# nyu-systems/CLM-GS

Measured on AMD Instinct MI355X. Metric: training images/s (Rubble-4K 28M Gaussians clm_offload), higher is better.
Workload: dtype f32

## Files before the change

### clm_gs_amd/_lib.py

```python
import ctypes
import os
import time

import torch

_HERE = os.path.dirname(os.path.abspath(__file__))
LIB_PATH = os.environ.get("CLMGS_LIB_PATH") or os.path.join(_HERE, "libclmgs_hip.so")

_vp, _i, _i64, _f, _sz = ctypes.c_void_p, ctypes.c_int, ctypes.c_int64, ctypes.c_float, ctypes.c_size_t
_d = ctypes.c_double

SIGNATURES = {
    "clmgs_version": (_i, []),
    "clmgs_last_error": (ctypes.c_char_p, []),
    "clmgs_projection_fwd": (_i, [_vp, _i, _i, _vp, _vp, _vp, _vp, _vp, _i, _i, _f, _f, _f, _f, _vp, _vp, _vp, _vp]),
    "clmgs_visibility_select_temp_bytes": (_sz, [_i, _i]),
    "clmgs_visibility_select_count": (_i, [_vp, _i, _i, _vp, _vp, _vp, _vp, _vp, _i, _i, _f, _f, _f, _f, _vp, _sz, _vp]),
    "clmgs_visibility_select_count_blocks": (_i, [_vp, _i, _i, _vp, _vp, _vp, _vp, _vp, _i, _i, _f, _f, _f, _f, _vp, _sz, _vp, _vp]),
    "clmgs_visibility_select_emit": (_i, [_vp, _i, _i, _vp, _vp]),
    "clmgs_visibility_raw": (_i, [_vp, _i, _i, _vp, _vp, _vp, _vp, _vp, _i, _i, _f, _f, _f, _f, _vp]),
    "clmgs_projection_bwd": (_i, [_vp, _i, _i, _vp, _vp, _vp, _vp, _vp, _i, _i, _f, _vp, _vp, _vp, _vp, _vp, _vp, _vp]),
    "clmgs_sh_fwd": (_i, [_vp, _i, _i, _vp, _vp, _vp, _vp]),
    "clmgs_sh_bwd": (_i, [_vp, _i, _i, _vp, _vp, _vp, _vp, _vp, _i, _vp]),
    "clmgs_isect_count_temp_bytes": (_sz, [_i]),
    "clmgs_isect_count": (_i, [_vp, _i, _i, _vp, _vp, _i, _i, _i, _vp, _vp, _vp, _sz]),
    "clmgs_isect_sort_temp_bytes": (_sz, [_i64]),
    "clmgs_isect_emit_sort": (_i, [_vp, _i, _i, _i64, _vp, _vp, _vp, _vp, _i, _i, _i, _vp, _vp, _vp, _sz]),
    "clmgs_isect_offsets": (_i, [_vp, _i64, _vp, _i, _i, _i, _vp]),
    "clmgs_isect2_order_temp_bytes": (_sz, [_i]),
    "clmgs_isect2_order_count": (_i, [_vp, _i, _vp, _vp, _vp, _i, _i, _i, _vp, _vp, _vp, _vp, _vp, _vp, _sz, _vp]),
    "clmgs_isect2_sort_temp_bytes": (_sz, [_i64]),
    "clmgs_isect2_emit_sort": (_i, [_vp, _i, _i64, _vp, _vp, _vp, _vp, _i, _i, _vp, _vp, _vp, _vp, _vp, _sz, _vp]),
    "clmgs_isect2_emit_sort_dev": (_i, [_vp, _i, _i64, _vp, _vp, _vp, _vp, _vp, _i, _i, _vp, _vp, _vp, _vp, _vp, _sz, _vp]),
    "clmgs_isect3_front_temp_bytes": (_sz, [_i, _i]),
    "clmgs_isect3_front": (_i, [_vp, _i, _vp, _vp, _i, _i, _i, _vp, _vp, _vp, _vp, _sz]),
    "clmgs_isect3_bin_temp_bytes": (_sz, [_i64, _i]),
    "clmgs_isect3_bin": (_i, [_vp, _i, _i64, _vp, _i, _i, _vp, _vp, _vp, _vp, _vp, _vp, _vp, _sz]),
    "clmgs_isect3_bin_dev": (_i, [_vp, _i, _i64, _vp, _vp, _i, _i, _vp, _vp, _vp, _vp, _vp, _vp, _vp, _sz]),
    "clmgs_rasterize_fwd_dev": (_i, [_vp, _i, _i, _i64, _vp, _vp, _i, _i, _i, _i, _i, _vp, _vp, _vp, _vp, _vp, _vp]),
    "clmgs_rasterize_bwd_dev": (_i, [_vp, _i, _i, _i64, _vp, _vp, _vp, _i, _i, _i, _i, _i, _vp, _vp, _vp, _vp, _vp, _vp, _vp, _vp, _vp]),
    "clmgs_rasterize_pack_bytes": (_sz, [_i, _i]),
    "clmgs_rasterize_fwd": (_i, [_vp, _i, _i, _i64, _vp, _vp, _vp, _vp, _vp, _i, _i, _i, _i, _i, _vp, _vp, _vp, _vp, _vp, _vp]),
    "clmgs_rasterize_partials_bytes": (_sz, [_i64]),
    "clmgs_rasterize_bwd": (_i, [_vp, _i, _i, _i64, _vp, _vp, _i, _i, _i, _i, _i, _vp, _vp, _vp, _vp, _vp, _vp, _vp, _vp, _vp, _vp, _vp, _vp, _vp, _vp]),
    "clmgs_rasterize4_fwd": (_i, [_vp, _i, _i, _i64, _vp, _vp, _vp, _vp, _vp, _i, _i, _i, _i, _i, _vp, _vp, _vp, _vp, _vp, _vp]),
    "clmgs_rasterize4_bwd": (_i, [_vp, _i, _i, _i64, _vp, _vp, _i, _i, _i, _i, _i, _vp, _vp, _vp, _vp, _vp, _vp, _vp, _vp, _vp, _vp, _vp, _vp, _vp, _vp]),
    "clmgs_preprocess_fwd": (_i, [_vp, _i, _vp, _vp, _vp, _vp, _vp, _vp, _i, _vp, _vp, _vp, _i, _i, _i, _f, _f, _f, _f, _vp, _vp, _vp, _vp, _vp, _vp, _vp, _vp]),
    "clmgs_preprocess_bwd": (_i, [_vp, _i, _vp, _vp, _vp, _vp, _vp, _vp, _i, _vp, _vp, _vp, _i, _i, _i, _f, _vp, _vp, _vp, _vp, _vp, _vp, _vp, _vp, _vp, _vp, _vp, _i, _vp, _vp, _vp, _vp, _i]),
    "clmgs_ssim_fwd": (_i, [_vp, _i, _i, _i, _i, _vp, _vp, _vp, _vp, _vp, _vp]),
    "clmgs_ssim_bwd": (_i, [_vp, _i, _i, _i, _i, _vp, _vp, _vp, _f, _vp, _vp, _vp, _vp]),
    "clmgs_loss_slots": (_i, []),
    "clmgs_l1_ssim_loss_fwd": (_i, [_vp, _i, _i, _vp, _i64, _i64, _i64, _vp, _vp, _vp, _vp, _vp]),
    "clmgs_l1_ssim_loss_bwd": (_i, [_vp, _i, _i, _vp, _i64, _i64, _i64, _vp, _vp, _f, _vp, _vp, _vp, _vp]),
    "clmgs_rows_gather": (_i, [_vp, _vp, _vp, _vp, _vp, _i, _i64, _i, _i]),
    "clmgs_rows_scatter_add": (_i, [_vp, _vp, _vp, _vp, _vp, _i, _i64, _i, _i]),
    "clmgs_scatter_to_bit": (_i, [_vp, _vp, _i, _vp, _i64, _i]),
    "clmgs_extract_ffs": (_i, [_vp, _vp, _i, _i64, _vp]),
    "clmgs_pair_overlap_count": (_i, [_vp, _vp, _i, _i64, _i, _vp]),
    "clmgs_set_signal": (_i, [_vp, _vp, _i, ctypes.c_int32]),
    "clmgs_adam_rows": (_i, [_vp, _vp, _vp, _vp, _vp, _vp, _i, _vp, _i64, _i, _vp, _d, _d, _d, _i, _i, _f, _i]),
    "clmgs_pack_small": (_i, [_vp, _i64, _vp, _vp, _vp, _vp, _vp]),
    "clmgs_adam_small_packed": (_i, [_vp, _i64, _vp, _vp, _vp, _vp, _vp, _vp, _d, _d, _d, _i, _i, _f, _vp, _i]),
    "clmgs_adam_catch_up": (_i, [_vp, _vp, _vp, _vp, _vp, _vp, _i, _i64, _i, _vp, _d, _d, _d, _i, _i, _i, _vp, _vp, _f, _i]),
    "clmgs_host_adam_rows": (_i, [_vp, _vp, _vp, _vp, _vp, _i64, _i, _vp, _d, _d, _d, _i, _i, _f, _i, _vp, _i]),
    "clmgs_host_pool_start": (_i, [_i]),
    "clmgs_host_usable_cpus": (_i, []),
    "clmgs_memcpy_async": (_i, [_vp, _vp, _vp, _sz, _i]),
    "clmgs_host_rows_prepare": (_i, [_vp, _vp, _vp, _vp, _vp, _vp, _vp, _i64, _i, _vp, _d, _d, _d, _i, _i, _i, _f, _i, _vp, _i]),
    "clmgs_densify_stats": (_i, [_vp, _i64, _vp, _vp, _vp, _i, _f, _f, _vp, _vp, _vp]),
    "clmgs_morton_order_temp_bytes": (_sz, [_i64]),
    "clmgs_morton_order": (_i, [_vp, _i64, _vp, _vp, _vp, _vp, _sz]),
    "clmgs_tsp_tour": (_i, [_i, _vp, _vp]),
    "clmgs_knn3_mean_dist2": (_i, [_vp, _i, _vp, _vp, _f, _f, _f, _f, _i, _i, _i, _i, _vp]),
    "clmgs_host_groups_temp_bytes": (_sz, [_i64]),
    "clmgs_host_groups": (_i, [_vp, _i64, _vp, _vp, _i, _i, _vp, _i, _vp, _vp, _vp, _vp, _vp, _sz]),
    "clmgs_publish_pack": (_i, [_vp, _vp, _vp, _vp, _vp, _i, _i64, _i64, _i64, _i]),
    "clmgs_visibility_candidates": (_i, [_vp, _i, _i, _i, _i, _vp, _vp, _vp, _vp, _i, _i, _f, _f, _f, _f, _f, _vp]),
    "clmgs_small_rows_scatter": (_i, [_vp, _i64, _vp, _vp, _vp, _vp, _vp, _vp, _vp]),
    "clmgs_adam_small_packed_range": (_i, [_vp, _i64, _i64, _i64, _vp, _vp, _vp, _vp, _vp, _vp, _d, _d, _d, _i, _i, _f, _vp, _i]),
    "clmgs_small_deferred_kmax": (_i, []),
    "clmgs_adam_small_deferred": (_i, [_vp, _i64, _vp, _vp, _vp, _vp, _vp, _vp, _vp, _i, _i, _vp, _vp, _vp, _vp, _d, _d, _d,
                                       _f, _i, _vp, _vp, _i, _i, _f, _f, _f, _i, _vp]),
    "clmgs_device_errors": (_i, [_vp, _i]),
    "clmgs_pinned_alloc": (_vp, [_sz]),
    "clmgs_pinned_free": (_i, [_vp]),
}

_lib = None

TIMING = None
STATS = {"n_isects": [], "n_emitted": [], "host_wait_s": 0.0}


class ClmgsError(RuntimeError):
    pass


class _Entry:

    def __init__(self, name, fn, takes_stream):
        self.name, self.fn, self.takes_stream = name, fn, takes_stream

    def __call__(self, *args):
        if TIMING is None or not self.takes_stream:
            return self.fn(*args)
        s, e = torch.cuda.Event(enable_timing=True), torch.cuda.Event(enable_timing=True)
        h = getattr(args[0], "value", args[0])
        st = torch.cuda.ExternalStream(h) if h else torch.cuda.current_stream()
        s.record(st)
        rc = self.fn(*args)
        e.record(st)
        TIMING.setdefault(self.name, []).append((s, e))
        return rc


class _Namespace:
    pass


_NO_STREAM = {"clmgs_version", "clmgs_loss_slots", "clmgs_small_deferred_kmax", "clmgs_isect3_front_temp_bytes",
              "clmgs_isect3_bin_temp_bytes", "clmgs_last_error", "clmgs_isect_count_temp_bytes",
              "clmgs_isect_sort_temp_bytes", "clmgs_host_groups_temp_bytes", "clmgs_isect2_order_temp_bytes", "clmgs_isect2_sort_temp_bytes", "clmgs_visibility_select_temp_bytes", "clmgs_rasterize_pack_bytes", "clmgs_rasterize_partials_bytes", "clmgs_host_adam_rows", "clmgs_host_pool_start", "clmgs_host_usable_cpus", "clmgs_host_rows_prepare", "clmgs_tsp_tour",
              "clmgs_pinned_alloc", "clmgs_pinned_free", "clmgs_device_errors"}


def timing_summary():
    out = {}
    for name, evs in (TIMING or {}).items():
        out[name] = (len(evs), sum(s.elapsed_time(e) for s, e in evs))
    return out


def lib():
    global _lib
    if _lib is None:
        if not os.path.exists(LIB_PATH):
            raise ClmgsError(
                f"{LIB_PATH} not found: build it with `python -c 'import __graft_entry__ as g; g.build()'` "
                "(make -C clm_gs_amd/csrc).  clm_gs_amd has no CPU/eager fallback."
            )
        l = ctypes.CDLL(LIB_PATH)
        ns = _Namespace()
        for name, (res, args) in SIGNATURES.items():
            fn = getattr(l, name)
            fn.restype = res
            fn.argtypes = args
            setattr(ns, name, _Entry(name, fn, name not in _NO_STREAM))
        _lib = ns
    return _lib


def check(rc):
    if rc != 0:
        msg = lib().clmgs_last_error()
        raise ClmgsError(f"libclmgs_hip error {rc}: {msg.decode() if msg else ''}")


def check_device_errors():
    bits = ctypes.c_uint32(0)
    check(lib().clmgs_device_errors(ctypes.byref(bits), 1))
    if bits.value & 4:
        raise ClmgsError("deferred small-attribute Adam: a block of rows was further behind than the recorded step history "
                         "(clmgs_adam_small_deferred, device error bit 4): its parameters are wrong")
    if bits.value:
        raise ClmgsError(f"device error word {bits.value}: no kernel of this library raises that value (4 is the only one "
                         "in use); the results since the last check cannot be trusted")


HOST_REGIONS = None
REGION_TRACE = None
_ROCTX = None


def roctx():
    global _ROCTX
    if _ROCTX is None:
        _ROCTX = False
        if os.environ.get("CLMGS_ROCTX") == "1":
            for name in ("librocprofiler-sdk-roctx.so", "libroctx64.so"):
                try:
                    l = ctypes.CDLL(name)
                    l.roctxRangePushA.argtypes = [ctypes.c_char_p]
                    l.roctxRangePushA.restype = ctypes.c_int
                    l.roctxRangePop.restype = ctypes.c_int
                    _ROCTX = l
                    break
                except (OSError, AttributeError):
                    continue
    return _ROCTX


class host_region:
    __slots__ = ("name", "t0", "rx")

    def __init__(self, name):
        self.name = name

    def __enter__(self):
        self.rx = roctx()
        if self.rx:
            self.rx.roctxRangePushA(self.name.encode())
        if HOST_REGIONS is not None:
            self.t0 = time.perf_counter()

    def __exit__(self, *exc):
        if HOST_REGIONS is not None:
            dt = time.perf_counter() - self.t0
            HOST_REGIONS[self.name] = HOST_REGIONS.get(self.name, 0.0) + dt
            if REGION_TRACE is not None:
                REGION_TRACE.setdefault(self.name, []).append(round(dt * 1e3, 2))
        if self.rx:
            self.rx.roctxRangePop()
        return False


def stream():
    return ctypes.c_void_p(torch.cuda.current_stream().cuda_stream)


def dptr(t, dtype=None, allow_none=False, allow_host=False):
    if t is None:
        if allow_none:
            return None
        raise ClmgsError("required tensor is None")
    if dtype is not None and t.dtype != dtype:
        raise ClmgsError(f"expected dtype {dtype}, got {t.dtype}")
    if not t.is_contiguous():
        raise ClmgsError("tensor must be contiguous")
    if not t.is_cuda:
        if not (allow_host and (t.is_pinned() or getattr(t, "_clmgs_pinned", False))):
            raise ClmgsError("tensor must live on the GPU (no CPU fallback in clm_gs_amd)")
    return ctypes.c_void_p(t.data_ptr())
```

### clm_gs_amd/clm_kernels.py

```python
import ctypes

import torch

from . import _lib, utils
from ._lib import check, dptr, stream

F32, I32, I64, U8 = torch.float32, torch.int32, torch.int64, torch.uint8


class _FusedSSIM(torch.autograd.Function):
    @staticmethod
    def forward(ctx, img1, img2):
        L = _lib.lib()
        img1, img2 = img1.contiguous(), img2.contiguous()
        B, CH, H, W = img1.shape
        need = img1.requires_grad
        ssim_sum = torch.zeros((1024,), dtype=F32, device=img1.device)
        maps = [torch.empty_like(img1) for _ in range(3)] if need else [None, None, None]
        check(L.clmgs_ssim_fwd(stream(), B, CH, H, W, dptr(img1, F32), dptr(img2, F32),
                               dptr(ssim_sum), dptr(maps[0], F32, True), dptr(maps[1], F32, True),
                               dptr(maps[2], F32, True)))
        ctx.shape = (B, CH, H, W)
        if need:
            ctx.save_for_backward(img1, img2, *maps)
        return ssim_sum.sum() / float(img1.numel())

    @staticmethod
    def backward(ctx, v):
        L = _lib.lib()
        img1, img2, m0, m1, m2 = ctx.saved_tensors
        B, CH, H, W = ctx.shape
        v_img1 = torch.empty_like(img1)
        v = v.reshape(1).to(F32).contiguous()
        check(L.clmgs_ssim_bwd(stream(), B, CH, H, W, dptr(img1), dptr(img2), dptr(v, F32),
                               1.0 / float(img1.numel()), dptr(m0), dptr(m1), dptr(m2),
                               dptr(v_img1)))
        return v_img1, None


def fused_ssim(img1, img2):
    return _FusedSSIM.apply(img1, img2)


class _FusedL1SSIMLoss(torch.autograd.Function):
    @staticmethod
    def forward(ctx, image, gt_u8, lambda_dssim):
        L = _lib.lib()
        assert image.dim() == 3 and image.shape[0] == 3 and image.dtype == F32 and image.is_cuda
        _, H, W = image.shape
        gt_u8 = gt_u8.contiguous()
        assert gt_u8.dtype == U8 and gt_u8.shape == image.shape
        need = image.requires_grad
        slots = L.clmgs_loss_slots()
        partials = torch.zeros((slots, 2), dtype=F32, device=image.device)
        maps = torch.empty((3, 3, H, W), dtype=F32, device=image.device) if need else None
        sc, sy, sx = image.stride()
        check(L.clmgs_l1_ssim_loss_fwd(stream(), H, W, ctypes.c_void_p(image.data_ptr()), sc, sy, sx,
                                       dptr(gt_u8, U8), dptr(partials),
                                       dptr(maps[0] if need else None, F32, True),
                                       dptr(maps[1] if need else None, F32, True),
                                       dptr(maps[2] if need else None, F32, True)))
        tot = partials.sum(dim=0) / float(image.numel())
        ctx.lam = float(lambda_dssim)
        if need:
            ctx.save_for_backward(image, gt_u8, maps)
        return (1.0 - ctx.lam) * tot[0] + ctx.lam * (1.0 - tot[1])

    @staticmethod
    def backward(ctx, v):
        L = _lib.lib()
        image, gt_u8, maps = ctx.saved_tensors
        _, H, W = image.shape
        v = v.reshape(1).to(F32).contiguous()
        v_img = torch.empty_strided(image.shape, image.stride(), dtype=F32, device=image.device)
        sc, sy, sx = image.stride()
        check(L.clmgs_l1_ssim_loss_bwd(stream(), H, W, ctypes.c_void_p(image.data_ptr()), sc, sy, sx,
                                       dptr(gt_u8, U8), dptr(v, F32), ctx.lam, dptr(maps[0]),
                                       dptr(maps[1]), dptr(maps[2]),
                                       ctypes.c_void_p(v_img.data_ptr())))
        return v_img, None, None


def fused_l1_ssim_loss(image, gt_u8, lambda_dssim=0.2):
    return _FusedL1SSIMLoss.apply(image, gt_u8, lambda_dssim)


def _idx64(t):
    return 1 if t is not None and t.dtype == I64 else 0


def _rows(fn, dst, src, dst_idx, src_idx, grid):
    L = _lib.lib()
    n = (dst_idx if dst_idx is not None else src_idx).numel() if (dst_idx is not None or src_idx is not None) else dst.shape[0]
    if dst_idx is not None and src_idx is not None and dst_idx.dtype != src_idx.dtype:
        src_idx = src_idx.to(dst_idx.dtype)
    is64 = _idx64(dst_idx if dst_idx is not None else src_idx)
    cols = src.shape[-1]
    check(getattr(L, fn)(stream(), dptr(dst, F32, allow_host=True), dptr(src, F32, allow_host=True),
                         dptr(dst_idx, None, True), dptr(src_idx, None, True), is64, int(n),
                         int(cols), int(grid)))


def send_shs2gpu_stream(shs, parameters, filter_idx, grid_size=0, block_size=256):
    _rows("clmgs_rows_gather", shs, parameters, None, filter_idx, grid_size)


def send_shs2gpu_stream_retention(shs_next, parameters, shs_retent, host_indices_to_param,
                                  rtnt_indices_to_param, param_indices_from_host,
                                  param_indices_from_rtnt, grid_size=0, block_size=256,
                                  grid_size_D=0, block_size_D=256):
    if host_indices_to_param.numel():
        _rows("clmgs_rows_gather", shs_next, parameters, param_indices_from_host,
              host_indices_to_param, grid_size)
    if rtnt_indices_to_param.numel():
        _rows("clmgs_rows_gather", shs_next, shs_retent, param_indices_from_rtnt,
              rtnt_indices_to_param, grid_size_D)


def send_shs2cpu_grad_buffer_stream(shs_grad, grad_buffer, filter_idx, accum=True, grid_size=0,
                                    block_size=256):
    _rows("clmgs_rows_scatter_add" if accum else "clmgs_rows_gather", grad_buffer, shs_grad,
          filter_idx, None, grid_size)


def send_shs2cpu_grad_buffer_stream_retention(shs_grad, grad_buffer, shs_grad_next,
                                              host_indices_from_grad, rtnt_indices_from_grad,
                                              grad_indices_to_host, grad_indices_to_rtnt,
                                              accum=True, grid_size=0, block_size=256,
                                              grid_size_D=0, block_size_D=256):
    if host_indices_from_grad.numel():
        _rows("clmgs_rows_scatter_add" if accum else "clmgs_rows_gather", grad_buffer, shs_grad,
              host_indices_from_grad, grad_indices_to_host, grid_size)
    if rtnt_indices_from_grad.numel():
        _rows("clmgs_rows_gather", shs_grad_next, shs_grad, rtnt_indices_from_grad,
              grad_indices_to_rtnt, grid_size_D)


@torch.no_grad()
def spherical_harmonics_bwd_inplace(degrees_to_use, dirs, coeffs, v_coeffs, v_colors):
    L = _lib.lib()
    n = dirs.numel() // 3
    d2, c2, vc = dirs.contiguous(), coeffs.contiguous(), v_colors.contiguous()
    v_dirs = torch.empty_like(d2)
    check(L.clmgs_sh_bwd(stream(), n, int(degrees_to_use), dptr(d2, F32), dptr(c2, F32), None,
                         dptr(vc, F32), dptr(v_coeffs, F32), 1, dptr(v_dirs)))
    return v_dirs


def scatter_to_bit(bitmap, filter_idx, bit):
    L = _lib.lib()
    check(L.clmgs_scatter_to_bit(stream(), dptr(bitmap), bitmap.element_size(),
                                 dptr(filter_idx.contiguous(), I64), filter_idx.numel(), int(bit)))


def extract_ffs(bitmap, ffs):
    L = _lib.lib()
    check(L.clmgs_extract_ffs(stream(), dptr(bitmap), bitmap.element_size(), bitmap.numel(),
                              dptr(ffs, U8)))


def compute_cnt_h(bitmap, tmp_buffer, grid_size=64, block_size=256):
    L = _lib.lib()
    bsz = tmp_buffer.shape[0] + 1
    cnt = torch.zeros((bsz - 1,), dtype=I32, device=bitmap.device)
    check(L.clmgs_pair_overlap_count(stream(), dptr(bitmap), bitmap.element_size(), bitmap.numel(),
                                     bsz, dptr(cnt)))
    tmp_buffer.zero_()
    tmp_buffer[:, 0] = cnt
    return cnt


def pair_overlap_count(bitmap, bsz):
    L = _lib.lib()
    cnt = torch.zeros((bsz - 1,), dtype=I32, device=bitmap.device)
    check(L.clmgs_pair_overlap_count(stream(), dptr(bitmap), bitmap.element_size(), bitmap.numel(),
                                     int(bsz), dptr(cnt)))
    return cnt


def set_signal(signal_tensor_pinned, idx, value):
    L = _lib.lib()
    check(L.clmgs_set_signal(stream(), ctypes.c_void_p(signal_tensor_pinned.data_ptr()), int(idx),
                             int(value)))


def selective_adam_update(param, grad, exp_avg, exp_avg_sq, visibility, lr, beta1, beta2, eps, N, M):
    L = _lib.lib()
    col_lr = torch.full((M,), float(lr), dtype=F32, device=param.device)
    vis = visibility.contiguous().view(U8)
    check(L.clmgs_adam_rows(stream(), dptr(param, F32), dptr(grad, F32), dptr(exp_avg, F32),
                            dptr(exp_avg_sq, F32), None, 0, dptr(vis, U8), int(N), int(M),
                            dptr(col_lr), float(beta1), float(beta2), float(eps), 1, 0, 1.0, 0))


def adam_rows(p, g, m, v, rows, col_lr, beta1, beta2, eps, step, bias_correction=True,
              grad_scale=1.0, zero_grad=False, mask=None):
    L = _lib.lib()
    n_rows = rows.numel() if rows is not None else p.shape[0]
    cols = p.shape[-1] if p.dim() > 1 else 1
    check(L.clmgs_adam_rows(stream(), dptr(p, F32), dptr(g, F32, True), dptr(m, F32), dptr(v, F32),
                            dptr(rows, None, True), _idx64(rows),
                            dptr(mask.view(U8) if mask is not None else None, U8, True),
                            int(n_rows), int(cols), dptr(col_lr, F32), float(beta1), float(beta2),
                            float(eps), int(step), int(bool(bias_correction)), float(grad_scale),
                            int(bool(zero_grad))))


def adam_catch_up(p, m, v, last_step, rows, col_lr, beta1, beta2, eps, to_step, bias_correction=True,
                  max_replay=256, g=None, g_step=None, grad_scale=1.0, keep_grad=False, moment_row0=0):
    L = _lib.lib()
    n_rows = rows.numel() if rows is not None else p.shape[0]
    m_ptr, v_ptr = dptr(m, F32), dptr(v, F32)
    if moment_row0:
        assert rows is not None, "a moment shard needs an explicit row list"
        back = int(moment_row0) * int(p.shape[-1]) * 4
        m_ptr, v_ptr = ctypes.c_void_p(m_ptr.value - back), ctypes.c_void_p(v_ptr.value - back)
    check(L.clmgs_adam_catch_up(stream(), dptr(p, F32), m_ptr, v_ptr, dptr(last_step, I32),
                                dptr(rows, None, True), _idx64(rows), int(n_rows), int(p.shape[-1]),
                                dptr(col_lr, F32), float(beta1), float(beta2), float(eps), int(to_step),
                                int(bool(bias_correction)), int(max_replay), dptr(g, F32, True),
                                dptr(g_step, I32, True), float(grad_scale), int(bool(keep_grad))))
    if rows is None:
        last_step[: p.shape[0]].fill_(int(to_step))
    else:
        utils.fill_rows(last_step, rows.long(), int(to_step))


def densify_stats(filter_idx, v_means2d, radii, width, height, max_radii2D, xyz_gradient_accum,
                  denom, only_visible=True):
    L = _lib.lib()
    n = radii.numel()
    check(L.clmgs_densify_stats(stream(), n, dptr(filter_idx, I64, True),
                                dptr(v_means2d.contiguous(), F32), dptr(radii.contiguous(), I32),
                                int(bool(only_visible)), float(width) * 0.5, float(height) * 0.5, dptr(max_radii2D, F32),
                                dptr(xyz_gradient_accum, F32), dptr(denom, F32)))
```

### clm_gs_amd/csrc/loss.hip

```cpp
#include "common.h"

namespace clmgs {

constexpr int LR = 5;
constexpr int LM = 2 * LR + 1;
constexpr int LS_W = 64, LS_ROWS = 62;
constexpr int LS_IN = LS_W + 2 * LR;
constexpr int LS_PITCH = LS_IN + 2;
constexpr int LS_RING = 8;
constexpr int LU = 12;
#ifndef CLMGS_LOSS_LP
#define CLMGS_LOSS_LP 4
#endif
constexpr int LP = CLMGS_LOSS_LP;
constexpr int LOSS_SLOTS = 1024;
constexpr float L_C1 = 0.01f * 0.01f, L_C2 = 0.03f * 0.03f;

constexpr float l_win[11] = {
    0.0010283801f, 0.0075987582f, 0.0360007721f, 0.1093606895f, 0.2130055377f, 0.2660117249f,
    0.2130055377f, 0.1093606895f, 0.0360007721f, 0.0075987582f, 0.0010283801f};

struct ImgView { const float* p; int64_t sc, sy, sx; };

__device__ __forceinline__ void wave_sync() {
  __builtin_amdgcn_fence(__ATOMIC_RELEASE, "wavefront");
  __builtin_amdgcn_wave_barrier();
  __builtin_amdgcn_fence(__ATOMIC_ACQUIRE, "wavefront");
}

__device__ __forceinline__ float gt_from_byte(unsigned byte) {
  const float v = (float)byte;
  const float r = 1.0f / 255.0f;
  const float q = v * r;
  return fmaf(fmaf(-q, 255.0f, v), r, q);
}

__device__ __forceinline__ bool strip_of_block(int H, int W, int& c, int& x0, int& y0, int& slot) {
  const int n_sx = (W + LS_W - 1) / LS_W, n_sy = (H + LS_ROWS - 1) / LS_ROWS;
  const int grp = blockIdx.x / 24, rem = blockIdx.x - grp * 24;
  c = rem >> 3;
  const int strip = grp * 8 + (rem & 7);
  if (strip >= n_sx * n_sy) return false;
  const int by = strip / n_sx, bx = strip - by * n_sx;
  x0 = bx * LS_W; y0 = by * LS_ROWS;
  slot = ((c * n_sy + by) * n_sx + bx) & (LOSS_SLOTS - 1);
  return true;
}

#ifndef CLMGS_LOSS_FWD_WAVES
#define CLMGS_LOSS_FWD_WAVES 3
#endif
__global__ void __launch_bounds__(64, CLMGS_LOSS_FWD_WAVES)
loss_fwd_kernel(int H, int W, ImgView img, const uint8_t* __restrict__ gt, float* __restrict__ partials,
                float* __restrict__ m1, float* __restrict__ m2, float* __restrict__ m3) {
  __shared__ float la[LS_RING][LS_PITCH], lb[LS_RING][LS_PITCH];
  const int lane = threadIdx.x;
  int c, x0, y0, slot;
  if (!strip_of_block(H, W, c, x0, y0, slot)) return;
  const size_t plane = (size_t)H * W;
  const int xo = x0 + lane;
  const int n_rows = min(LS_ROWS, H - y0) + 2 * LR;
  const int xs = x0 - LR + lane;
  const bool xs_ok = xs >= 0 && xs < W;
  const int xh = x0 - LR + LS_W + lane;
  const bool h_ok = lane < 2 * LR && xh < W;
  const float* img_c = img.p + c * img.sc;
  const uint8_t* gt_c = gt + c * plane;
  const unsigned xs_c = (unsigned)min(max(xs, 0), W - 1);
  const unsigned xh_c = (unsigned)min(x0 - LR + LS_W + min(lane, 2 * LR - 1), W - 1);
  const unsigned xs_off = xs_c * (unsigned)img.sx, xh_off = xh_c * (unsigned)img.sx;
  float pa[LP], ha[LP];
  unsigned pb[LP], hb[LP];
  auto fetch = [&](int r, int s) {
    const int y = min(max(y0 - LR + min(r, n_rows - 1), 0), H - 1);
    const float* ir = img_c + y * img.sy;
    const uint8_t* gr = gt_c + (size_t)y * W;
    pa[s] = ir[xs_off]; pb[s] = gr[xs_c];
    ha[s] = ir[xh_off]; hb[s] = gr[xh_c];
  };
#pragma unroll
  for (int s = 0; s < LP; ++s) fetch(s, s);
  float win[LU][4];
  float l1 = 0.f, ss = 0.f;
  for (int r0 = 0; r0 < n_rows; r0 += LU) {
#pragma unroll
    for (int k = 0; k < LU; ++k) {
      const int r = r0 + k;
      {
        __builtin_amdgcn_sched_barrier(0);
        const int s = k % LP, buf = r & (LS_RING - 1);
        {
          const int yin = y0 - LR + r;
          const bool row_ok = yin >= 0 && yin < H;
          const bool okm = row_ok && xs_ok, okh = row_ok && h_ok;
          la[buf][lane] = okm ? pa[s] : 0.f; lb[buf][lane] = okm ? gt_from_byte(pb[s]) : 0.f;
          if (lane < 2 * LR) {
            la[buf][LS_W + lane] = okh ? ha[s] : 0.f; lb[buf][LS_W + lane] = okh ? gt_from_byte(hb[s]) : 0.f;
          }
        }
        fetch(r + LP, s);
        wave_sync();
        float s0 = 0.f, s1 = 0.f, s2 = 0.f, s3 = 0.f;
#pragma unroll
        for (int j = 0; j < LM; ++j) {
          const float av = la[buf][lane + j], bv = lb[buf][lane + j];
          const float wa_ = l_win[j] * av, wb_ = l_win[j] * bv;
          s0 += wa_; s1 += wb_; s2 = fmaf(wa_, av, s2); s2 = fmaf(wb_, bv, s2); s3 = fmaf(wa_, bv, s3);
        }
        win[k][0] = s0; win[k][1] = s1; win[k][2] = s2; win[k][3] = s3;
        {
          float acc[4];
#pragma unroll
          for (int q = 0; q < 4; ++q) {
            float sacc = 0.f;
#pragma unroll
            for (int j = 0; j < LM; ++j) sacc += l_win[j] * win[(k + 2 + j) % LU][q];
            acc[q] = sacc;
          }
          const int y = y0 + r - 2 * LR;
          const bool out_ok = (r >= 2 * LR) && (r < n_rows) && (xo < W) && (y < H);
          {
            const float mu1 = acc[0], mu2 = acc[1];
            const float mu1sq = mu1 * mu1, mu2sq = mu2 * mu2, mu12 = mu1 * mu2;
            const float sgs = (acc[2] - mu1sq) - mu2sq, sg12 = acc[3] - mu12;
            const float A = 2.f * mu12 + L_C1, B = 2.f * sg12 + L_C2;
            const float D = mu1sq + mu2sq + L_C1, E = sgs + L_C2;
            const float iDE = __builtin_amdgcn_rcpf(D * E);
            const float val = A * B * iDE;
            ss += out_ok ? val : 0.f;
            const int cbuf = (r - LR) & (LS_RING - 1);
            l1 += out_ok ? fabsf(la[cbuf][lane + LR] - lb[cbuf][lane + LR]) : 0.f;
            if (m1 && out_ok) {
              const float d_mu1 = 2.f * mu2 * B * iDE - val * 2.f * mu1 * __builtin_amdgcn_rcpf(D);
              const float d_s1 = -val * __builtin_amdgcn_rcpf(E), d_s12 = 2.f * A * iDE;
              const size_t orow = c * plane + (size_t)y * W;
              (m1 + orow)[(unsigned)xo] = d_mu1 - 2.f * mu1 * d_s1 - mu2 * d_s12;
              (m2 + orow)[(unsigned)xo] = d_s1; (m3 + orow)[(unsigned)xo] = d_s12;
            }
          }
        }
      }
    }
  }
  const float tl1 = wave_sum(l1), tss = wave_sum(ss);
  if (lane == 0) {
    atomicAdd(partials + 2 * slot, tl1);
    atomicAdd(partials + 2 * slot + 1, tss);
  }
}

#ifndef CLMGS_LOSS_BWD_WAVES
#define CLMGS_LOSS_BWD_WAVES 3
#endif
__global__ void __launch_bounds__(64, CLMGS_LOSS_BWD_WAVES)
loss_bwd_kernel(int H, int W, ImgView img, const uint8_t* __restrict__ gt, const float* __restrict__ v,
                float w_l1_over_numel, float w_ssim_over_numel, const float* __restrict__ m1,
                const float* __restrict__ m2, const float* __restrict__ m3, float* __restrict__ v_img,
                int64_t vsc, int64_t vsy, int64_t vsx) {
  __shared__ float lm[2][3][LS_PITCH];
  const int lane = threadIdx.x;
  int c, x0, y0, slot;
  if (!strip_of_block(H, W, c, x0, y0, slot)) return;
  const size_t plane = (size_t)H * W;
  const int xo = x0 + lane;
  const int n_out = min(LS_ROWS, H - y0);
  const int n_rows = n_out + 2 * LR;
  const int xs = x0 - LR + lane;
  const bool xs_ok = xs >= 0 && xs < W;
  const int hg = lane >> 4, hl = lane & 15;
  const int xh = x0 - LR + LS_W + hl;
  const bool h_ok = hg < 3 && hl < 2 * LR && xh < W;
  const float* mh = (hg == 0 ? m1 : (hg == 1 ? m2 : m3)) + c * plane;
  const float* m1c = m1 + c * plane;
  const float* m2c = m2 + c * plane;
  const float* m3c = m3 + c * plane;
  const float* img_c = img.p + c * img.sc;
  const uint8_t* gt_c = gt + c * plane;
  const float vv = v[0];
  const unsigned xs_c = (unsigned)min(max(xs, 0), W - 1);
  const unsigned xh_c = (unsigned)min(x0 - LR + LS_W + min(hl, 2 * LR - 1), W - 1);
  const unsigned xo_c = (unsigned)min(xo, W - 1);
  const unsigned xo_off = xo_c * (unsigned)img.sx;
  const unsigned xo_voff = (unsigned)xo * (unsigned)vsx;
  float p1[LP], p2[LP], p3[LP], ph[LP], px[LP];
  unsigned py[LP];
  auto fetch = [&](int r, int s) {
    const int rc = min(r, n_rows - 1);
    const int y = min(max(y0 - LR + rc, 0), H - 1);
    const int yo = min(max(y0 + rc - 2 * LR, 0), H - 1);
    const size_t o = (size_t)y * W;
    p1[s] = (m1c + o)[xs_c]; p2[s] = (m2c + o)[xs_c]; p3[s] = (m3c + o)[xs_c];
    ph[s] = (mh + o)[xh_c];
    px[s] = (img_c + yo * img.sy)[xo_off];
    py[s] = (gt_c + (size_t)yo * W)[xo_c];
  };
#pragma unroll
  for (int s = 0; s < LP; ++s) fetch(s, s);
  float win[LU][3];
  for (int r0 = 0; r0 < n_rows; r0 += LU) {
#pragma unroll
    for (int k = 0; k < LU; ++k) {
      const int r = r0 + k;
      {
        __builtin_amdgcn_sched_barrier(0);
        const int s = k % LP, buf = r & 1;
        {
          const int yin = y0 - LR + r;
          const bool row_ok = yin >= 0 && yin < H;
          const bool okm = row_ok && xs_ok;
          lm[buf][0][lane] = okm ? p1[s] : 0.f; lm[buf][1][lane] = okm ? p2[s] : 0.f; lm[buf][2][lane] = okm ? p3[s] : 0.f;
          if (hg < 3 && hl < 2 * LR) lm[buf][hg][LS_W + hl] = (row_ok && h_ok) ? ph[s] : 0.f;
        }
        const float xv = px[s], yv = gt_from_byte(py[s]);
        fetch(r + LP, s);
        wave_sync();
        float s0 = 0.f, s1 = 0.f, s2 = 0.f;
#pragma unroll
        for (int j = 0; j < LM; ++j) {
          s0 = fmaf(l_win[j], lm[buf][0][lane + j], s0);
          s1 = fmaf(l_win[j], lm[buf][1][lane + j], s1);
          s2 = fmaf(l_win[j], lm[buf][2][lane + j], s2);
        }
        win[k][0] = s0; win[k][1] = s1; win[k][2] = s2;
        {
          float g[3];
#pragma unroll
          for (int q = 0; q < 3; ++q) {
            float sacc = 0.f;
#pragma unroll
            for (int j = 0; j < LM; ++j) sacc += l_win[j] * win[(k + 2 + j) % LU][q];
            g[q] = sacc;
          }
          const int y = y0 + r - 2 * LR;
          if (r >= 2 * LR && r < n_rows && xo < W) {
            const float sgn = (xv > yv) ? 1.f : ((xv < yv) ? -1.f : 0.f);
            const float dss = g[0] + 2.f * xv * g[1] + yv * g[2];
            (v_img + (c * vsc + y * vsy))[xo_voff] = vv * (w_l1_over_numel * sgn - w_ssim_over_numel * dss);
          }
        }
        wave_sync();
      }
    }
  }
}

}

using namespace clmgs;

extern "C" int clmgs_loss_slots(void) { return LOSS_SLOTS; }

extern "C" int clmgs_l1_ssim_loss_fwd(void* stream, int H, int W, const float* img, int64_t stride_c,
                                      int64_t stride_y, int64_t stride_x, const uint8_t* gt_u8,
                                      float* partials, float* m1, float* m2, float* m3) {
  CLMGS_CHECK_ARG(H >= 1 && W >= 1 && img && gt_u8 && partials);
  CLMGS_CHECK_ARG((m1 && m2 && m3) || (!m1 && !m2 && !m3));
  ImgView v{img, stride_c, stride_y, stride_x};
  const int64_t strips = (int64_t)ceil_div(W, LS_W) * ceil_div(H, LS_ROWS);
  dim3 grid((unsigned)(24 * ceil_div(strips, 8)));
  hipLaunchKernelGGL(loss_fwd_kernel, grid, dim3(64), 0, (hipStream_t)stream, H, W, v, gt_u8,
                     partials, m1, m2, m3);
  CLMGS_LAUNCH_CHECK();
  return 0;
}

extern "C" int clmgs_l1_ssim_loss_bwd(void* stream, int H, int W, const float* img, int64_t stride_c,
                                      int64_t stride_y, int64_t stride_x, const uint8_t* gt_u8,
                                      const float* v_loss, float lambda_dssim, const float* m1,
                                      const float* m2, const float* m3, float* v_img) {
  CLMGS_CHECK_ARG(H >= 1 && W >= 1 && img && gt_u8 && v_loss && m1 && m2 && m3 && v_img);
  ImgView v{img, stride_c, stride_y, stride_x};
  const double numel = 3.0 * (double)H * (double)W;
  const int64_t strips = (int64_t)ceil_div(W, LS_W) * ceil_div(H, LS_ROWS);
  dim3 grid((unsigned)(24 * ceil_div(strips, 8)));
  hipLaunchKernelGGL(loss_bwd_kernel, grid, dim3(64), 0, (hipStream_t)stream, H, W, v, gt_u8, v_loss,
                     (float)((1.0 - lambda_dssim) / numel), (float)(lambda_dssim / numel), m1, m2, m3,
                     v_img, stride_c, stride_y, stride_x);
  CLMGS_LAUNCH_CHECK();
  return 0;
}
```

### clm_gs_amd/fused.py

```python
import ctypes
import math

import numpy as np
import torch

from . import _lib, utils
from ._lib import check, dptr
from .gsplat import (_record_counts, bucket_size, empty_bucketed, isect2_begin, isect2_counts, isect2_finish, isect3_begin,
                     isect3_finish)

F32, I32, U8 = torch.float32, torch.int32, torch.uint8
TILE = 16


def _partial_line_floats():
    global _PART_FLOATS
    if _PART_FLOATS is None:
        _PART_FLOATS = int(_lib.lib().clmgs_rasterize_partials_bytes(1)) // 4
    return _PART_FLOATS


_PART_FLOATS = None


def _cam_host(camera):
    h = getattr(camera, "_clmgs_host", None)
    if h is None:
        vm = camera.world_view_transform.detach().t().contiguous().cpu().numpy().astype(np.float32)
        K = camera.K.detach().cpu().numpy().astype(np.float32) if getattr(camera, "K", None) is not None \
            else camera.create_k_on_gpu().cpu().numpy().astype(np.float32)
        c2w = getattr(camera, "camtoworlds", None)
        if c2w is not None:
            campos = c2w.detach().reshape(-1, 4, 4)[0, :3, 3].cpu().numpy().astype(np.float32)
        else:
            campos = np.linalg.inv(vm.astype(np.float64))[:3, 3].astype(np.float32)
        h = (np.ascontiguousarray(vm.reshape(16)), np.ascontiguousarray(K.reshape(9)),
             np.ascontiguousarray(campos.reshape(3)))
        camera._clmgs_host = h
    return h


def _np(a):
    return a.ctypes.data_as(ctypes.c_void_p)


class _CameraPass:
    __slots__ = ("V", "cam", "filt", "sh_rows", "sh_by_filter", "small_in", "small_packed", "radii",
                 "packed", "fids", "offsets", "emit_slot", "row_cum", "out", "alphas", "last_ids",
                 "bg", "v_out", "maps", "loss", "ev_loss", "streams", "deg", "aux", "loss_partials",
                 "lambda_dssim", "gt_u8", "background", "isect", "sh_index", "means2d", "n_dev")


def _sptr(torch_stream):
    return ctypes.c_void_p(torch_stream.cuda_stream)


_CAPACITY = {}
_CAP_HELD = {}
_CAP_IDS = __import__("itertools").count(1)


def _cap_key(gaussians, W, H):
    k = getattr(gaussians, "_clmgs_cap_id", None)
    if k is None:
        k = gaussians._clmgs_cap_id = next(_CAP_IDS)
    return (int(W), int(H), k)


def _observe_count(key, n):
    _CAPACITY[key] = max(int(n), int(0.98 * _CAPACITY.get(key, 0)))


def _capacity_for(key, args):
    seen = _CAPACITY.get(key)
    if not seen or not getattr(args, "device_side_counts", True):
        return None
    margin = float(getattr(args, "isect_capacity_margin", 1.25))
    floor = int(getattr(args, "isect_capacity_floor", 4096))
    held = _CAP_HELD.get(key)
    if held is not None and margin > 1.0 and int(seen * 1.10) + floor <= held <= int(seen * margin * 1.5) + floor:
        return held
    cap = int(seen * margin) + floor
    cap = bucket_size(cap) if cap > 4096 else max(cap, 1)
    _CAP_HELD[key] = cap
    return cap


def camera_forward(gaussians, camera, this_filter, sh_rows, sh_by_filter, background, gt_u8,
                   lambda_dssim=0.2, small_packed=None, streams=None, sh_index=None, exact=True):
    return camera_forward_finish(gaussians, camera_front(
        gaussians, camera, this_filter, sh_rows, sh_by_filter, background, gt_u8, lambda_dssim,
        small_packed, streams, sh_index), exact=exact)


def camera_front(gaussians, camera, this_filter, sh_rows, sh_by_filter, background, gt_u8,
                 lambda_dssim=0.2, small_packed=None, streams=None, sh_index=None):
    L = _lib.lib()
    args = utils.get_args()
    W, H = int(utils.get_img_width()), int(utils.get_img_height())
    dev = gaussians._xyz.device
    cur = torch.cuda.current_stream()
    s_front, s_mem, s_raster = streams if streams is not None else (cur, cur, cur)
    p = _CameraPass()
    p.streams = (s_front, s_mem, s_raster)
    V = p.V = int(this_filter.shape[0]) if this_filter is not None else int(gaussians._xyz.shape[0])
    p.cam = _cam_host(camera)
    vm, K, campos = p.cam
    deg = p.deg = int(gaussians.active_sh_degree)
    p.sh_rows, p.sh_by_filter, p.small_packed = sh_rows, sh_by_filter, small_packed
    p.sh_index = sh_index
    p.gt_u8, p.lambda_dssim, p.background = gt_u8, float(lambda_dssim), background
    filt = p.filt = this_filter.contiguous() if this_filter is not None else None
    if small_packed is not None:
        small_in = (dptr(small_packed, F32), None, None, None)
        p.aux = (small_packed,)
    else:
        xyz, opa = gaussians._xyz.detach(), gaussians._opacity.detach()
        sca, rot = gaussians._scaling.detach(), gaussians._rotation.detach()
        small_in = (dptr(xyz, F32), dptr(opa, F32), dptr(sca, F32), dptr(rot, F32))
        p.aux = (xyz, opa, sca, rot)
    p.small_in = small_in
    tw, th = math.ceil(W / float(TILE)), math.ceil(H / float(TILE))
    with torch.cuda.stream(s_front):
        radii = p.radii = empty_bucketed(V, (), I32, dev).reshape(1, V)
        means2d = empty_bucketed(V, (2,), F32, dev).reshape(1, V, 2)
        depths = empty_bucketed(V, (), F32, dev).reshape(1, V)
        packed = p.packed = empty_bucketed(V, (16,), F32, dev)
        check(L.clmgs_preprocess_fwd(
            _sptr(s_front), V, dptr(filt, torch.int64, True), *small_in,
            dptr(sh_rows, F32, allow_host=True), int(sh_by_filter), _np(vm), _np(K), _np(campos), W, H, deg,
            0.3, 0.01, 1e10, float(getattr(args, "radius_clip", 0.0)), dptr(radii), dptr(means2d),
            dptr(depths), None, None, None, dptr(packed),
            dptr(sh_index, I32, True)))
        begin = isect3_begin if getattr(args, "binning", "tile") == "tile" else isect2_begin
        p.isect = begin(means2d, radii, depths, TILE, tw, th, want_slots=True,
                        packed=packed if getattr(args, "exact_tile_cull", True) else None)
        p.aux = p.aux + (means2d, depths)
        p.means2d = means2d
    return p


def camera_forward_finish(gaussians, p, exact=False):
    L = _lib.lib()
    args = utils.get_args()
    W, H = int(utils.get_img_width()), int(utils.get_img_height())
    dev = gaussians._xyz.device
    s_front, s_mem, s_raster = p.streams
    V, packed, background, gt_u8, lambda_dssim = p.V, p.packed, p.background, p.gt_u8, p.lambda_dssim
    tw, th = math.ceil(W / float(TILE)), math.ceil(H / float(TILE))
    cap = None if (exact or V == 0) else _capacity_for(_cap_key(gaussians, W, H), args)
    with torch.cuda.stream(s_front):
        with _lib.host_region("fwd_isect"):
            finish = isect3_finish if p.isect.route == "tile" else isect2_finish
            p.fids, p.offsets, _, (p.emit_slot, p.row_cum) = finish(p.isect, capacity=cap)
        if cap is None:
            p.isect, p.n_dev = None, None
            if V:
                _observe_count(_cap_key(gaussians, W, H), p.fids.numel())
        else:
            p.n_dev = p.isect.totals
        p.out = torch.empty((H, W, 3), dtype=F32, device=dev)
        p.alphas = torch.empty((H, W), dtype=F32, device=dev)
        p.last_ids = torch.empty((H, W), dtype=I32, device=dev)
        p.bg = background.reshape(1, 3).to(F32).contiguous() if background is not None else None
    if s_raster is not s_front:
        s_raster.wait_stream(s_front)
    n_isects = p.fids.numel()
    if p.n_dev is None:
        check(L.clmgs_rasterize_fwd(_sptr(s_raster), 1, V, n_isects, None, None, None, None, dptr(p.bg, F32, True),
                                    W, H, TILE, tw, th, dptr(p.offsets), dptr(p.fids), dptr(packed), dptr(p.out),
                                    dptr(p.alphas), dptr(p.last_ids)))
    else:
        check(L.clmgs_rasterize_fwd_dev(_sptr(s_raster), 1, V, n_isects, dptr(p.n_dev), dptr(p.bg, F32, True),
                                        W, H, TILE, tw, th, dptr(p.offsets), dptr(p.fids), dptr(packed), dptr(p.out),
                                        dptr(p.alphas), dptr(p.last_ids)))
    if s_mem is not s_raster:
        ev = torch.cuda.Event()
        ev.record(s_raster)
        s_mem.wait_event(ev)
    with torch.cuda.stream(s_mem):
        slots = L.clmgs_loss_slots()
        partials = torch.zeros((slots, 2), dtype=F32, device=dev)
        maps = p.maps = torch.empty((3, 3, H, W), dtype=F32, device=dev)
        sc, sy, sx = 1, 3 * W, 3
        gt = gt_u8.contiguous()
        sm = _sptr(s_mem)
        check(L.clmgs_l1_ssim_loss_fwd(sm, H, W, dptr(p.out), sc, sy, sx, dptr(gt, U8), dptr(partials),
                                       dptr(maps[0]), dptr(maps[1]), dptr(maps[2])))
        p.loss_partials, p.loss = partials, None
        one = getattr(gaussians, "_clmgs_one", None)
        if one is None or one.device != dev:
            one = gaussians._clmgs_one = torch.ones((1,), dtype=F32, device=dev)
        p.v_out = torch.empty_like(p.out)
        check(L.clmgs_l1_ssim_loss_bwd(sm, H, W, dptr(p.out), sc, sy, sx, dptr(gt, U8), dptr(one),
                                       float(lambda_dssim), dptr(maps[0]), dptr(maps[1]), dptr(maps[2]),
                                       dptr(p.v_out)))
        p.ev_loss = None
        if s_raster is not s_mem:
            p.ev_loss = torch.cuda.Event()
            p.ev_loss.record(s_mem)
        p.aux = p.aux + (gt, one, partials)
        p.maps = None
        del maps
    return p


def camera_loss(p):
    if p.loss is None:
        W, H = int(utils.get_img_width()), int(utils.get_img_height())
        tot = p.loss_partials.sum(dim=0) / float(3 * H * W)
        p.loss = ((1.0 - p.lambda_dssim) * tot[0] + p.lambda_dssim * (1.0 - tot[1])).detach()
    return p.loss


def camera_verify(gaussians, p):
    c = p.isect
    if c is None or p.n_dev is None:
        return
    W, H = int(utils.get_img_width()), int(utils.get_img_height())
    n, n_ref = isect2_counts(c)
    _observe_count(_cap_key(gaussians, W, H), n)
    if n <= p.fids.numel():
        _record_counts(n, n_ref)
        p.isect = None
        return
    _lib.STATS["isect_capacity_redo"] = _lib.STATS.get("isect_capacity_redo", 0) + 1
    for st in set(p.streams):
        st.synchronize()
    p.n_dev = None
    camera_forward_finish(gaussians, p, exact=True)


def camera_backward(gaussians, p, g_sh_rows, small_grad=None, update_stats=True, stats_delta=None,
                    stats_only_visible=False, visibility_out=None, accumulate_after=None, sh_stamp=None,
                    cur_step=0, release=False):
    L = _lib.lib()
    args = utils.get_args()
    W, H = int(utils.get_img_width()), int(utils.get_img_height())
    dev = gaussians._xyz.device
    camera_verify(gaussians, p)
    s_front, s_mem, s_raster = p.streams
    V = p.V
    vm, K, campos = p.cam
    tw, th = math.ceil(W / float(TILE)), math.ceil(H / float(TILE))
    n_isects = p.fids.numel()
    if p.small_packed is not None:
        assert small_grad is not None
        small_out = (dptr(small_grad, F32), None, None, None)
    else:
        small_out = (dptr(gaussians._xyz.grad, F32), dptr(gaussians._opacity.grad, F32),
                     dptr(gaussians._scaling.grad, F32), dptr(gaussians._rotation.grad, F32))
    with torch.cuda.stream(s_raster):
        partials = empty_bucketed(max(n_isects, 1), (_partial_line_floats(),), F32, dev)
    if p.ev_loss is not None:
        s_raster.wait_event(p.ev_loss)
    if p.n_dev is None:
        check(L.clmgs_rasterize_bwd(_sptr(s_raster), 1, V, n_isects, dptr(p.packed), dptr(p.bg, F32, True), W, H,
                                    TILE, tw, th, dptr(p.offsets), dptr(p.fids), dptr(p.alphas), dptr(p.last_ids),
                                    dptr(p.v_out), None, None, None, None, None, None,
                                    dptr(p.emit_slot), dptr(p.row_cum), dptr(partials)))
    else:
        check(L.clmgs_rasterize_bwd_dev(_sptr(s_raster), 1, V, n_isects, dptr(p.n_dev), dptr(p.packed),
                                        dptr(p.bg, F32, True), W, H, TILE, tw, th, dptr(p.offsets), dptr(p.fids),
                                        dptr(p.alphas), dptr(p.last_ids), dptr(p.v_out), None,
                                        dptr(p.emit_slot), dptr(p.row_cum), dptr(partials)))
    if s_mem is not s_raster:
        ev = torch.cuda.Event()
        ev.record(s_raster)
        s_mem.wait_event(ev)
    stats = update_stats and (not args.disable_auto_densification) and \
        utils.get_cur_iter() <= args.densify_until_iter
    if stats and stats_delta is not None:
        stat_ptrs = (dptr(stats_delta, F32), None, None)
    else:
        stat_ptrs = (dptr(gaussians.max_radii2D if stats else None, F32, True),
                     dptr(gaussians.xyz_gradient_accum if stats else None, F32, True),
                     dptr(gaussians.denom if stats else None, F32, True))
    with torch.cuda.stream(s_mem):
        if accumulate_after is not None:
            s_mem.wait_event(accumulate_after)
        if visibility_out is not None:
            visibility_out |= (p.radii.reshape(-1) > 0)
        check(L.clmgs_preprocess_bwd(
            _sptr(s_mem), V, dptr(p.filt, torch.int64, True), *p.small_in, dptr(p.sh_rows, F32, allow_host=True),
            int(p.sh_by_filter), _np(vm), _np(K), _np(campos), W, H, p.deg, 0.3, dptr(p.radii),
            None, *small_out, dptr(g_sh_rows, F32, allow_host=True),
            *stat_ptrs, None, int(bool(stats_only_visible)), dptr(partials), dptr(p.row_cum),
            dptr(p.sh_index, I32, True), dptr(sh_stamp, I32, True), int(cur_step)))
    if s_mem is not s_raster:
        partials.record_stream(s_mem)
        p.v_out.record_stream(s_raster)
    del partials
    p.v_out = None
    if release:
        for name in ("radii", "packed", "fids", "offsets", "emit_slot", "row_cum", "out", "alphas", "last_ids", "n_dev"):
            t = getattr(p, name)
            if t is not None:
                for st in {s_mem, s_raster} - {s_front}:
                    t.record_stream(st)
                setattr(p, name, None)
        for t in p.aux:
            if isinstance(t, torch.Tensor) and t.is_cuda and t is not p.loss_partials:
                for st in {s_mem, s_raster} - {s_front}:
                    t.record_stream(st)
        p.aux = (p.loss_partials,)
        p.means2d = None
    return p


def train_one_camera(gaussians, camera, this_filter, sh_rows, sh_by_filter, g_sh_rows, background,
                     gt_u8, lambda_dssim=0.2, update_stats=True, keep=None, accumulate_after=None,
                     return_event=False, stats_only_visible=False, visibility_out=None,
                     raster_stream=None, small_packed=None, small_grad=None, stats_delta=None, sh_index=None,
                     sh_stamp=None, cur_step=0):
    cur = torch.cuda.current_stream()
    p = camera_forward(gaussians, camera, this_filter, sh_rows, sh_by_filter, background, gt_u8,
                       lambda_dssim, small_packed, (cur, cur, raster_stream if raster_stream is not None else cur),
                       sh_index, exact=False)
    camera_backward(gaussians, p, g_sh_rows, small_grad, update_stats, stats_delta,
                    stats_only_visible, visibility_out, accumulate_after, sh_stamp, cur_step)
    loss = camera_loss(p)
    if keep is not None:
        keep.append(p)
    if return_event:
        ev = torch.cuda.Event()
        ev.record(cur)
        return loss, ev
    return loss
```

### clm_gs_amd/strategies/clm_offload/engine.py

```python
import math
import os

import torch

from ... import _lib, clm_kernels, dp, fast_tsp, utils
from ...clm_kernels import (send_shs2cpu_grad_buffer_stream, send_shs2gpu_stream,
                            spherical_harmonics_bwd_inplace)
from ...densification import update_densification_stats_offload_accum_grads
from ...gsplat import (fully_fused_projection, isect_offset_encode, isect_tiles,
                       rasterize_to_pixels, spherical_harmonics)
from ...host import pinned_empty
from ..base_engine import (select_filters, TILE_SIZE, calculate_filters, pipeline_forward_one_step,
                           torch_compiled_loss)

_BITMAP_DTYPE = {4: torch.int8, 8: torch.int8, 16: torch.int16, 32: torch.int32, 64: torch.int64}


def pipeline_forward_one_step_shs_inplace(filtered_opacity_gpu, filtered_scaling_gpu,
                                          filtered_rotation_gpu, filtered_xyz_gpu, filtered_shs,
                                          camera, scene, gaussians, background, pipe_args):
    viewmat = camera.world_view_transform.transpose(0, 1)
    K = camera.K
    n_selected = filtered_xyz_gpu.shape[0]
    image_width, image_height = int(utils.get_img_width()), int(utils.get_img_height())
    radiis, means2D, depths, conics, _ = fully_fused_projection(
        means=filtered_xyz_gpu, covars=None, quats=filtered_rotation_gpu,
        scales=filtered_scaling_gpu, viewmats=viewmat.unsqueeze(0), Ks=K.unsqueeze(0),
        width=image_width, height=image_height, packed=False)
    means2D.retain_grad()
    dirs = filtered_xyz_gpu[None, :, :] - camera.camtoworlds[:, None, :3, 3]
    filtered_shs = filtered_shs.reshape(1, n_selected, 16, 3)
    with torch.no_grad():
        colors_origin = spherical_harmonics(degrees_to_use=gaussians.active_sh_degree, dirs=dirs,
                                            coeffs=filtered_shs)
    colors_detached = colors_origin.detach().requires_grad_()
    colors = torch.clamp_min(colors_detached + 0.5, 0.0)
    opacities = filtered_opacity_gpu.squeeze(1).unsqueeze(0)
    tile_width = math.ceil(image_width / float(TILE_SIZE))
    tile_height = math.ceil(image_height / float(TILE_SIZE))
    _, isect_ids, flatten_ids = isect_tiles(means2d=means2D, radii=radiis, depths=depths,
                                            tile_size=TILE_SIZE, tile_width=tile_width,
                                            tile_height=tile_height, packed=False)
    isect_offsets = isect_offset_encode(isect_ids, 1, tile_width, tile_height)
    backgrounds = background.reshape(1, 3) if background is not None else None
    rendered_image, _ = rasterize_to_pixels(
        means2d=means2D, conics=conics, colors=colors, opacities=opacities,
        image_width=image_width, image_height=image_height, tile_size=TILE_SIZE,
        isect_offsets=isect_offsets, flatten_ids=flatten_ids, backgrounds=backgrounds)
    rendered_image = rendered_image.squeeze(0).permute(2, 0, 1)
    return rendered_image, means2D, radiis, colors_detached, dirs


def _encode_bitmap(filters, n_gaussians, bsz):
    bitmap = torch.zeros((n_gaussians,), dtype=_BITMAP_DTYPE[bsz], device=filters[0].device)
    for i, f in enumerate(filters):
        clm_kernels.scatter_to_bit(bitmap, f, bsz - 1 - i)
    return bitmap


def finish_groups(filters, n_gaussians, bsz, sparse_adam=False):
    dev = filters[0].device
    bitmap = _encode_bitmap(filters, n_gaussians, bsz)
    ffs = torch.empty(n_gaussians, dtype=torch.uint8, device=dev)
    clm_kernels.extract_ffs(bitmap, ffs)
    groups = [torch.nonzero(ffs == 0).flatten()]
    for mb in range(bsz):
        groups.append(torch.nonzero(ffs == (bsz - mb)).flatten())
    visibility_mask = (ffs != 0) if sparse_adam else None
    cnt_d = clm_kernels.pair_overlap_count(bitmap, bsz).tolist()
    lens = [len(f) for f in filters]
    cnt_h = [lens[i + 1] - cnt_d[i] for i in range(bsz - 1)]
    cnt_g = [lens[i] - cnt_d[i] for i in range(bsz - 1)]
    return groups, visibility_mask, cnt_h, cnt_d, cnt_g, bitmap


def order_calculation(filters, batched_cameras, n_gaussians, bsz, perm_generator, args):
    if bsz not in _BITMAP_DTYPE:
        raise ValueError("Currently supported bsz: (4, 8, 16, 32, 64).")
    dev = filters[0].device
    bitmap = _encode_bitmap(filters, n_gaussians, bsz)
    stride = bsz * bsz if bsz >= 32 else 32
    sample = bitmap[::stride].to(torch.int64)
    shifts = torch.arange(bsz - 1, -1, -1, device=dev)
    unz = ((sample[None, :] >> shifts[:, None]) & 1).to(torch.float32)
    ones = unz.sum(dim=1)
    inter = unz @ unz.t()
    distance_matrix = (ones[:, None] + ones[None, :] - 2 * inter).round().to(torch.int64).tolist()
    ordered_cams = fast_tsp.find_tour(distance_matrix, 0.001)
    if args.reorder_by_min_sparsity_at_end:
        k_min = bsz - 1
        for k in range(bsz - 1):
            if len(filters[ordered_cams[k]]) < len(filters[ordered_cams[k_min]]):
                k_min = k
        ordered_cams = ordered_cams[k_min + 1:] + ordered_cams[:k_min + 1]
    batched_cameras = [batched_cameras[i] for i in ordered_cams]
    filters = [filters[i] for i in ordered_cams]
    sparsity = [len(f) / float(n_gaussians) for f in filters]

    groups, visibility_mask, cnt_h, cnt_d, cnt_g, bitmap = finish_groups(filters, n_gaussians, bsz, args.sparse_adam)

    sizes = [g.numel() for g in groups]
    cat = torch.cat(groups).to(torch.int32)
    cat_h = pinned_empty((max(cat.numel(), 1),), dtype=torch.int32)[:cat.numel()]
    cat_h.copy_(cat)
    finish_indices_filters = list(torch.split(cat_h, sizes))
    assert len(finish_indices_filters) == bsz + 1
    assert sum(sizes) == n_gaussians, (sum(sizes), n_gaussians)
    return (finish_indices_filters, batched_cameras, filters, sparsity, ordered_cams, cnt_h, cnt_d,
            cnt_g, visibility_mask, bitmap)


def _gather_small(gaussians, this_filter):
    idx = this_filter
    xyz = gaussians._xyz.detach()[idx].requires_grad_(True)
    opa = gaussians._opacity.detach()[idx].requires_grad_(True)
    sca = gaussians._scaling.detach()[idx].requires_grad_(True)
    rot = gaussians._rotation.detach()[idx].requires_grad_(True)
    return xyz, opa, sca, rot


def _scatter_small_grads(gaussians, this_filter, xyz, opa, sca, rot):
    with torch.no_grad():
        gaussians._xyz.grad.index_add_(0, this_filter, xyz.grad)
        gaussians._opacity.grad.index_add_(0, this_filter, opa.grad)
        gaussians._scaling.grad.index_add_(0, this_filter, sca.grad)
        gaussians._rotation.grad.index_add_(0, this_filter, rot.grad)


def _render_and_backward(gaussians, scene, camera, background, pipe_args, this_filter, shs,
                         shs_grad, before_sh_backward=None):
    if getattr(utils.get_args(), "fused_front_end", True):
        from ...fused import train_one_camera
        if before_sh_backward is not None:
            before_sh_backward()
        return train_one_camera(gaussians, camera, this_filter, shs, 0, shs_grad, background,
                                camera.original_image)
    xyz, opa_raw, sca_raw, rot_raw = _gather_small(gaussians, this_filter)
    opa = gaussians.opacity_activation(opa_raw)
    sca = gaussians.scaling_activation(sca_raw)
    rot = gaussians.rotation_activation(rot_raw)
    image, means2D, radiis, colors_detached, dirs = pipeline_forward_one_step_shs_inplace(
        opa, sca, rot, xyz, shs, camera, scene, gaussians, background, pipe_args)
    loss = torch_compiled_loss(image, camera.original_image)
    loss.backward()
    if before_sh_backward is not None:
        before_sh_backward()
    v_dirs = spherical_harmonics_bwd_inplace(
        degrees_to_use=gaussians.active_sh_degree, dirs=dirs, coeffs=shs.reshape(1, -1, 16, 3),
        v_coeffs=shs_grad, v_colors=colors_detached.grad)
    dirs.backward(v_dirs)
    _scatter_small_grads(gaussians, this_filter, xyz, opa_raw, sca_raw, rot_raw)
    update_densification_stats_offload_accum_grads(
        scene, gaussians, int(utils.get_img_height()), int(utils.get_img_width()), this_filter,
        means2D.grad.squeeze(0), radiis.squeeze(0))
    return loss.detach()


def _zero_small_grads(gaussians):
    clean = getattr(gaussians, "_clean_grad_ptrs", ())
    for p in (gaussians._xyz, gaussians._opacity, gaussians._scaling, gaussians._rotation):
        g = p.grad
        if g is None or g.shape != p.shape or g.data_ptr() not in clean:
            p.grad = torch.zeros_like(p)
    gaussians._clean_grad_ptrs = ()


def _gpu_adam_step(gaussians, args, visibility_mask, grad_div=None):
    grad_div = float(grad_div or args.bsz)
    small = gaussians.all_parameters()[:4]
    if args.stop_update_param or args.sparse_adam:
        for param in small:
            if param.grad is not None:
                param.grad /= grad_div
        if not args.stop_update_param:
            gaussians.optimizer.gpu_adam.step(visibility=visibility_mask)
        gaussians.optimizer.gpu_adam.zero_grad(set_to_none=True)
        return
    gaussians.optimizer.gpu_step_scaled(1.0 / grad_div)
    gaussians._clean_grad_ptrs = tuple(p.grad.data_ptr() for p in small if p.grad is not None)


def _pipeline_streams(gaussians):
    sts = getattr(gaussians, "_clmgs_streams", None)
    if sts is None:
        try:
            lo, hi = torch.cuda.Stream.priority_range()
        except AttributeError:
            lo, hi = 0, -1
        sts = gaussians._clmgs_streams = {
            "aux": torch.cuda.Stream(),
            "mem": [torch.cuda.Stream(priority=hi) for _ in range(2)],
            "raster": [torch.cuda.Stream(priority=lo) for _ in range(2)]}
    return sts


def reserve_working_set(gaussians, n_cameras_in_flight=2):
    W, H = int(utils.get_img_width()), int(utils.get_img_height())
    P, N = W * H, int(gaussians._xyz.shape[0])
    I = int(1.0 * P)
    V = min(N, max(1, N // 6))
    k = int(n_cameras_in_flight)
    sts = _pipeline_streams(gaussians)
    plan = {
        "front": (sts["mem"][0], k * (20 * P + 70 * I + 96 * V)),
        "mem": (sts["mem"][1], k * 48 * P + (1 << 20)),
        "raster": (sts["raster"][0], 2 * k * 64 * int(0.8 * I)),
        "default": (torch.cuda.current_stream(), 240 * N + 64 * V * 4),
    }
    out = {}
    try:
        free_now = torch.cuda.mem_get_info(gaussians._xyz.device)[0]
    except Exception:
        free_now = None
    total = sum(int(nb) for _, nb in plan.values())
    shrink = 1.0 if not free_now or total <= free_now / 3 else (free_now / 3) / total
    for name, (st, nbytes) in plan.items():
        nbytes = int(nbytes * shrink)
        if nbytes < (1 << 20):
            out[name] = 0
            continue
        try:
            with torch.cuda.stream(st):
                blk = torch.empty((nbytes,), dtype=torch.uint8, device=gaussians._xyz.device)
                small = [torch.empty((1 << 19,), dtype=torch.uint8, device=gaussians._xyz.device) for _ in range(16)]
                del blk, small
            out[name] = nbytes
        except torch.cuda.OutOfMemoryError:
            torch.cuda.empty_cache()
            out[name] = 0
    return out


class _Batch:
    """State of one HBM-resident batch, handed from stage to stage (see _train_one_batch_hbm)."""


def _stage_visibility(b):
    gaussians, args, cams = b.gaussians, b.args, b.cameras
    N = b.N
    b.touched = b.touched_rows = None
    b.small_owner = bool(getattr(gaussians, "small_owner", False) and gaussians.lazy_rows and dp.active()
                         and not args.stop_update_param)
    if b.small_owner:
        with torch.no_grad(), _lib.host_region("dp_small_fetch"), dp.phase("S"):
            gaussians.small_prepare(cams)
    b.small_deferred = bool(getattr(gaussians, "small_deferred", False) and b.fused and gaussians.lazy_rows
                            and not args.stop_update_param and getattr(args, "packed_small", True))
    blk_flags = None
    if b.small_deferred:
        with torch.no_grad():
            blk_flags = gaussians.small_catch_up(cams)
    with torch.no_grad():
        if b.fused:
            with _lib.host_region("select_filters"):
                b.filters, b.touched_rows = select_filters(cams, gaussians._xyz.detach(), gaussians._scaling.detach(),
                                                           gaussians._rotation.detach(), block_flags=blk_flags)
        else:
            b.filters, _, _ = calculate_filters(cams, gaussians.get_xyz, gaussians.get_opacity,
                                                gaussians.get_scaling, gaussians.get_rotation)
    if b.small_owner and os.environ.get("CLMGS_DP_DEBUG") and b.touched_rows is not None:
        lo_, hi_ = dp.owner_range(N)
        foreign = b.touched_rows[(b.touched_rows < lo_) | (b.touched_rows >= hi_)]
        cand_ = getattr(gaussians, "_dbg_cand", None)
        miss = -1
        if cand_ is not None and gaussians._small_since > 0:
            isc = torch.zeros((N,), dtype=torch.bool, device=foreign.device)
            isc[cand_] = True
            miss = int((~isc[foreign]).sum())
        print("DPDEBUG batch rank %d since %d foreign touched rows %d not candidates %d" % (
            dp.rank(), gaussians._small_since, foreign.numel(), miss), flush=True)
        assert miss <= 0
    b.sparsity = [len(f) / float(N) for f in b.filters]
    b.ordered_cams = list(range(b.bsz))
    if getattr(args, "reference_camera_order", False):
        _, b.cameras, b.filters, b.sparsity, b.ordered_cams = order_calculation(
            list(b.filters), list(cams), N, b.bsz, None, args)[:5]


def _stage_plan(b):
    gaussians, args, N, bsz = b.gaussians, b.args, b.N, b.bsz
    b.lazy = gaussians.lazy_rows and not args.stop_update_param
    mode = getattr(args, "overlap_cameras", True)
    b.pipelined = b.fused and mode in (True, "pipeline")
    b.use_packed = (b.fused and getattr(args, "packed_small", True) and not args.sparse_adam
                    and not args.stop_update_param)
    b.locality = bool(b.lazy and dp.active() and getattr(args, "dp_locality", False))
    b.locality_sparse = bool(dp.active() and getattr(args, "dp_locality", False) and args.sparse_adam and b.fused
                             and not args.stop_update_param and not b.lazy)
    if getattr(args, "dp_locality", False) and dp.active():
        assert b.touched_rows is not None and (b.locality_sparse or (b.locality and b.use_packed and gaussians.first_touch_grads)), (
            "dp_locality needs the fused front end and either the dense deferred row optimizer with the packed "
            "small-attribute tables and first-touch gradient stores (defaults) or sparse_adam")
    need_mask = b.touched_rows is None or args.sparse_adam or (dp.active() and not b.locality) or not b.lazy
    if need_mask:
        b.touched = torch.zeros((N,), dtype=torch.bool, device=gaussians._xyz.device)
        if b.touched_rows is not None:
            utils.fill_rows(b.touched, b.touched_rows, True)
        else:
            for f in b.filters:
                utils.fill_rows(b.touched, f, True)
        if dp.active() and not b.locality_sparse:
            b.local_touched = b.touched
            b.touched = dp.allreduce_touched(b.touched)
            b.touched_rows = None
    b.row_adam = gaussians.optimizer.cpu_adam
    b.params = gaussians._parameters
    b.grad_buf = b.parameters_grad_buffer[:N]
    b.params.grad = b.grad_buf
    b.row_adam.global_step += 1
    b.step = b.row_adam.global_step
    _mark_batch(gaussians)
    b.group = b.row_adam.param_groups[0]
    b.st = b.row_adam.state[b.params]
    b.default_stream = torch.cuda.current_stream()
    b.side_event = None
    b.col_lr = b.row_adam._col_lr(b.params.device)
    if b.touched_rows is None:
        b.touched_rows = torch.nonzero(b.touched).flatten()
    b.touched_rows = b.touched_rows.to(torch.int32)
    _lib.STATS.setdefault("touched_rows", []).append(int(b.touched_rows.shape[0]))
    b.ft_stamp = gaussians._row_g_step if (b.lazy and b.fused and gaussians.first_touch_grads) else None


def _mark_batch(gaussians):
    gaussians._lazy_dirty = True
    gaussians._mutations = getattr(gaussians, "_mutations", 0) + 1
    gaussians._sorted_tag = None


def _row_update(b, rows, zero_grad_rows=False):
    clm_kernels.adam_rows(b.params.data, None if zero_grad_rows else b.grad_buf, b.st["exp_avg"],
                          b.st["exp_avg_sq"], rows, b.col_lr,
                          b.group["betas"][0], b.group["betas"][1], b.group["eps"], b.step,
                          b.group["bias_correction"], 1.0 / (b.bsz * dp.world_size()), True)


def _stage_exchange_head(b):
    gaussians, args, N, bsz, step = b.gaussians, b.args, b.N, b.bsz, b.step
    params, touched_rows = b.params, b.touched_rows
    b.owner = b.border = None
    b.split_catch = False
    b.dp_ev_b0 = b.dp_ev_b1 = b.dp_comm = None
    b.dp_split = False
    if b.locality:
        b.dp_split = bool(b.pipelined and bsz >= 2 and getattr(args, "dp_overlap", True))
        with _lib.host_region("dp_border_plan"), dp.phase("plan"):
            b.border = dp.border_plan(touched_rows.long(), N, first_rows=b.filters[0] if b.dp_split else None,
                                      last_rows=b.filters[bsz - 1] if b.dp_split else None,
                                      publish_counts=not b.small_owner)
        gaussians._owner_dirty = True
        own_rows = b.border.own_rows
        if own_rows.numel():
            with dp.phase("catch_up_own"):
                gaussians.catch_up_rows(own_rows.to(torch.int32), to_step=step - 1)
        if b.dp_split:
            b.dp_comm = getattr(gaussians, "_dp_comm_stream", None)
            if b.dp_comm is None:
                b.dp_comm = gaussians._dp_comm_stream = torch.cuda.Stream()
            b.dp_comm.wait_stream(b.default_stream)
            with torch.cuda.stream(b.dp_comm):
                with dp.phase("B0"):
                    dp.border_params_out(params.data, b.border, "params0")
                b.dp_ev_b0 = torch.cuda.Event()
                b.dp_ev_b0.record(b.dp_comm)
                with dp.phase("B1"):
                    dp.border_params_out(params.data, b.border, "params1")
                b.dp_ev_b1 = torch.cuda.Event()
                b.dp_ev_b1.record(b.dp_comm)
        else:
            with dp.phase("B"):
                dp.border_params_out(params.data, b.border)
    elif b.locality_sparse:
        with _lib.host_region("dp_border_plan"), dp.phase("plan"):
            b.border = dp.border_plan(touched_rows.long(), N)
        gaussians._owner_dirty = True
        with dp.phase("B"):
            dp.border_params_out(params.data, b.border)
    elif b.lazy and dp.active() and getattr(args, "dp_owner_computes", False):
        b.owner = dp.owner_plan(touched_rows.long(), N)
        gaussians._owner_dirty = True
        own_rows = touched_rows[b.owner.lo:b.owner.hi]
        if b.owner.hi > b.owner.lo:
            gaussians.catch_up_rows(own_rows, to_step=step - 1)
        dp.owner_gather_rows(params.data, b.owner)
    elif b.lazy:
        if (b.pipelined and bsz >= 2 and getattr(args, "split_catch_up", True) and b.filters is not None):
            b.foreign_rows = None
            if dp.active():
                lt = getattr(b, "local_touched", None)
                assert lt is not None
                b.foreign_rows = touched_rows[~lt[touched_rows.long()]]
            b.split_catch = True
            s_front = _pipeline_streams(gaussians)["mem"][0]
            s_front.wait_stream(b.default_stream)
            b.first_catch_done = bool(getattr(args, "early_first_catch_up", True))
            if b.first_catch_done and b.filters[0].numel():
                with torch.cuda.stream(s_front):
                    gaussians.catch_up_rows(b.filters[0], to_step=step - 1)
        else:
            gaussians.catch_up_rows(touched_rows, to_step=step - 1)
    elif not args.stop_update_param and not args.sparse_adam:
        untouched_rows = torch.nonzero(~b.touched).flatten().to(torch.int32)
        b.comm_stream.wait_stream(b.default_stream)
        with torch.cuda.stream(b.comm_stream):
            _row_update(b, untouched_rows, zero_grad_rows=True)
            b.side_event = torch.cuda.Event()
            b.side_event.record(b.comm_stream)
        untouched_rows.record_stream(b.comm_stream)


def _cameras_pipelined(b):
    from ...fused import camera_backward, camera_forward_finish, camera_front, camera_loss
    gaussians, bsz, step = b.gaussians, b.bsz, b.step
    sts = _pipeline_streams(gaussians)
    s_front, s_mem, s_raster = sts["mem"][0], sts["mem"][1], sts["raster"][0]
    if getattr(gaussians, "_clmgs_one", None) is None:
        gaussians._clmgs_one = torch.ones((1,), dtype=torch.float32, device=b.params.device)
    for st_ in (s_front, s_mem, s_raster):
        st_.wait_stream(b.default_stream)
    gaussians._clmgs_passes = None
    passes = []
    dp_recv0 = [None]

    def backward(k):
        with _lib.host_region("camera_backward"):
            camera_backward(gaussians, passes[k], b.grad_buf, b.small_gk, stats_delta=b.stats_d,
                            sh_stamp=b.ft_stamp, cur_step=step, release=True)
        if b.dp_split and k == bsz - 2:
            ev = torch.cuda.Event()
            ev.record(s_mem)
            b.dp_comm.wait_event(ev)
            with torch.cuda.stream(b.dp_comm), dp.phase("D0"):
                dp_recv0[0] = dp.border_grads_send([b.grad_buf, b.small_gk], b.ft_stamp, step, b.border, "grads0")

    def catch(k):
        if b.filters[k].numel():
            with torch.cuda.stream(s_front):
                gaussians.catch_up_rows(b.filters[k], to_step=step - 1)
    for k in range(bsz):
        if b.dp_split:
            s_front.wait_event(b.dp_ev_b0 if k == 0 else b.dp_ev_b1)
        if b.split_catch and (k or not b.first_catch_done):
            catch(k)
        if b.split_catch and k == bsz - 1 and getattr(b, "foreign_rows", None) is not None and b.foreign_rows.numel():
            with torch.cuda.stream(s_front):
                gaussians.catch_up_rows(b.foreign_rows, to_step=step - 1)
        with _lib.host_region("camera_front"):
            cur_pass = camera_front(gaussians, b.cameras[k], b.filters[k], b.params.data, 1, b.background,
                                    b.cameras[k].original_image, small_packed=b.small_pk,
                                    streams=(s_front, s_mem, s_raster))
        with _lib.host_region("camera_forward"):
            passes.append(camera_forward_finish(gaussians, cur_pass))
        if k >= 1:
            backward(k - 1)
    backward(bsz - 1)
    if b.dp_split:
        b.default_stream.wait_stream(b.dp_comm)
        gaussians._dp_recv0 = dp_recv0[0]
    for st_ in (s_front, s_mem, s_raster):
        b.default_stream.wait_stream(st_)
    losses = [camera_loss(p_) for p_ in passes]
    gaussians._clmgs_passes = passes
    return losses


def _stage_cameras(b):
    gaussians, args, bsz = b.gaussians, b.args, b.bsz
    b.small_pk = b.small_gk = b.stats_d = None
    if b.use_packed:
        b.small_pk, b.small_gk = gaussians.small_packed(), gaussians.small_grad()
        if (getattr(args, "packed_stats", True) and (not args.disable_auto_densification)
                and utils.get_cur_iter() <= args.densify_until_iter):
            b.stats_d = gaussians.stats_delta()
    else:
        _zero_small_grads(gaussians)
    if b.pipelined:
        return _cameras_pipelined(b)
    losses = []
    if b.fused:
        from ...fused import train_one_camera
        for k in range(bsz):
            losses.append(train_one_camera(
                gaussians, b.cameras[k], b.filters[k], b.params.data, 1, b.grad_buf, b.background,
                b.cameras[k].original_image, small_packed=b.small_pk, small_grad=b.small_gk,
                stats_delta=b.stats_d, sh_stamp=b.ft_stamp, cur_step=b.step))
        return losses
    for k in range(bsz):
        this_filter = b.filters[k]
        with torch.no_grad():
            shs = torch.empty((this_filter.shape[0], 48), device=b.params.device)
            send_shs2gpu_stream(shs, b.params.data, this_filter)
            shs_grad = torch.zeros_like(shs)
        loss = _render_and_backward(gaussians, b.scene, b.cameras[k], b.background, b.pipe_args, this_filter, shs,
                                    shs_grad)
        with torch.no_grad():
            send_shs2cpu_grad_buffer_stream(shs_grad, b.grad_buf, this_filter, True)
        losses.append(loss)
    return losses


def _stage_exchange_tail(b):
    if not dp.active():
        return
    gaussians, N, step = b.gaussians, b.N, b.step
    grad_buf, small_gk, ft_stamp, border = b.grad_buf, b.small_gk, b.ft_stamp, b.border
    if border is not None and b.locality_sparse:
        small_grads = [gaussians._xyz.grad, gaussians._opacity.grad, gaussians._scaling.grad, gaussians._rotation.grad]
        dp.border_grads_home([grad_buf] + small_grads, None, 0, border)
        own_rows = border.own_rows
        _, got = dp.publish_rows(small_grads, own_rows, N, counts=border.own_counts)
        b.touched = torch.zeros((N,), dtype=torch.bool, device=b.params.device)
        for ids in [own_rows] + got:
            if ids.numel():
                utils.fill_rows(b.touched, ids, True)
        b.touched_rows = own_rows.to(torch.int32)
    elif border is not None:
        if b.dp_split:
            r0 = gaussians._dp_recv0
            gaussians._dp_recv0 = None
            for t_ in (r0[0], r0[1], r0[3]):
                if isinstance(t_, torch.Tensor) and t_.is_cuda:
                    t_.record_stream(b.default_stream)
            with dp.phase("D1"):
                r1 = dp.border_grads_send([grad_buf, small_gk], ft_stamp, step, border, "grads1")
            with dp.phase("D_apply"):
                dp.border_grads_apply([grad_buf, small_gk], ft_stamp, step, border, r0)
                dp.border_grads_apply([grad_buf, small_gk], ft_stamp, step, border, r1)
        else:
            with dp.phase("D"):
                dp.border_grads_home([grad_buf, small_gk], ft_stamp, step, border)
        if not b.small_owner:
            dp.publish_small(small_gk, ft_stamp, step, N, border)
    elif b.owner is not None:
        if b.use_packed:
            dp.allreduce_tables_rows([small_gk], b.touched_rows, N, average=False)
        else:
            dp.allreduce_small_grads([gaussians._xyz.grad, gaussians._opacity.grad,
                                      gaussians._scaling.grad, gaussians._rotation.grad], average=False)
        dp.owner_reduce_rows(grad_buf, b.owner)
    elif b.use_packed:
        with dp.phase("allreduce"):
            dp.allreduce_tables_rows([small_gk, grad_buf], b.touched_rows, N, average=False)
    else:
        dp.allreduce_small_grads([gaussians._xyz.grad, gaussians._opacity.grad,
                                  gaussians._scaling.grad, gaussians._rotation.grad], average=False)
        dp.allreduce_rows(grad_buf, b.touched, average=False, rows=b.touched_rows)


def _stage_optimizer(b):
    gaussians, args, N, bsz, step = b.gaussians, b.args, b.N, b.bsz, b.step
    if b.use_packed and b.small_deferred and b.ft_stamp is not None and not dp.active():
        gaussians.small_defer_record(step)
    elif b.use_packed:
        if getattr(gaussians, "small_deferred", False):
            gaussians.flush_small()
        gaussians.optimizer.gpu_step_packed(b.small_pk, b.small_gk, 1.0 / (bsz * dp.world_size()),
                                            g_stamp=b.ft_stamp, cur_step=step,
                                            row_range=dp.owner_range(N) if (b.small_owner and b.locality) else None)
        if b.small_owner and b.locality:
            gaussians.small_after_step()
    else:
        _gpu_adam_step(gaussians, args, b.touched if args.sparse_adam else None,
                       grad_div=bsz * dp.world_size())
        gaussians.invalidate_small_packed()
    if b.lazy:
        stamp = b.touched_rows[b.owner.lo:b.owner.hi] if b.owner is not None else b.touched_rows
        if stamp.numel() and b.ft_stamp is None:
            utils.fill_rows(gaussians._row_g_step, stamp.long(), step)
    elif not args.stop_update_param:
        _row_update(b, b.touched_rows)
    b.st["step"] = step


def _train_one_batch_hbm(gaussians, scene, batched_cameras, parameters_grad_buffer, background,
                         pipe_args, comm_stream, args):
    b = _Batch()
    b.gaussians, b.scene, b.cameras, b.args = gaussians, scene, batched_cameras, args
    b.parameters_grad_buffer, b.background, b.pipe_args, b.comm_stream = parameters_grad_buffer, background, pipe_args, comm_stream
    b.bsz, b.N = len(batched_cameras), gaussians._xyz.shape[0]
    b.fused = bool(getattr(args, "fused_front_end", True))
    _stage_visibility(b)
    _stage_plan(b)
    _stage_exchange_head(b)
    losses = _stage_cameras(b)
    with dp.phase("tail_exchange"):
        _stage_exchange_tail(b)
    if getattr(args, "debug_skip_optimizer", False):
        b.row_adam.global_step -= 1
        if b.side_event is not None:
            b.default_stream.wait_event(b.side_event)
        return losses, b.ordered_cams, b.sparsity
    _stage_optimizer(b)
    if b.side_event is not None:
        b.default_stream.wait_event(b.side_event)
    if getattr(args, "sync_each_batch", False):
        torch.cuda.synchronize()
    return losses, b.ordered_cams, b.sparsity


def _bit_of(bitmap, ids, bit):
    return ((bitmap[ids].to(torch.int64) >> bit) & 1).to(torch.bool)


_HOST_CHUNK_ROWS = 262144


def _host_tables(gaussians, dev):
    N = gaussians._xyz.shape[0]
    ht = getattr(gaussians, "_host_tabs", None)
    if ht is None or ht["N"] != N:
        ht = gaussians._host_tabs = dict(N=N, slot_of=torch.zeros((N,), dtype=torch.int32, device=dev),
                                         mark=torch.zeros((N,), dtype=torch.bool, device=dev),
                                         in_spec=torch.zeros((N,), dtype=torch.bool, device=dev))
    return ht


def _host_buffers(gaussians, T, dev):
    from ...gsplat import bucket_size
    hb = getattr(gaussians, "_host_bufs", None)
    N = gaussians._xyz.shape[0]
    if hb is None or hb["cap"] < T or hb["N"] != N:
        cap = bucket_size(max(int(T * 1.08), 1))
        gen = hb["gen"] + 1 if hb else 0
        keep_pinned = None
        if hb is not None:
            torch.cuda.synchronize()
            if hb["N"] == N and hb["rows_h"].shape[0] >= cap:
                keep_pinned = (hb["rows_h"], hb["stage_h"], hb["spec_rows_h"], hb["spec_stage_h"])
            hb.clear()
        gaussians._host_bufs = None
        if keep_pinned is None:
            cap_h = bucket_size(max(int(T * 1.5), cap))
            keep_pinned = (pinned_empty((cap_h,), dtype=torch.int32), pinned_empty((cap_h, 48)), None, None)
        hb = gaussians._host_bufs = dict(
            cap=cap, N=N, cur=0, gen=gen,
            rows_h=keep_pinned[0], stage_h=keep_pinned[1], spec_rows_h=keep_pinned[2], spec_stage_h=keep_pinned[3],
            sh_stage=[torch.empty((cap, 48), device=dev), None],
            g_stage=torch.empty((cap, 48), device=dev))
    return hb


def _host_spec_buffers(hb, dev):
    if hb["sh_stage"][1] is None:
        hb["sh_stage"][1] = torch.empty((hb["cap"], 48), device=dev)
    if hb["spec_rows_h"] is None:
        cap_h = hb["rows_h"].shape[0]
        hb["spec_rows_h"] = pinned_empty((cap_h,), dtype=torch.int32)
        hb["spec_stage_h"] = pinned_empty((cap_h, 48))


def hint_next_batch(gaussians, cameras):
    gaussians._next_batch_hint = list(cameras) if cameras else None


def _drop_speculation(gaussians):
    gaussians.drop_host_speculation()


def _train_one_batch_host(gaussians, scene, batched_cameras, parameters_grad_buffer, background,
                          pipe_args, comm_stream, perm_generator, args):
    if getattr(args, "host_staging", "window") == "window":
        from .host_window import train_one_batch_host_windowed as run
    else:
        from .host_batch import train_one_batch_host_batched as run
    return run(gaussians, scene, batched_cameras, parameters_grad_buffer, background, pipe_args, comm_stream,
               perm_generator, args)


def clm_offload_train_one_batch(gaussians, scene, batched_cameras, parameters_grad_buffer,
                                background, pipe_args, comm_stream, perm_generator):
    args = utils.get_args()
    bsz = len(batched_cameras)
    assert bsz > 1 and bsz in _BITMAP_DTYPE, "clm_offload supports bsz in (4, 8, 16, 32, 64)"
    assert bsz == args.bsz, f"batch of {bsz} cameras but args.bsz = {args.bsz} (optimizer hyper-parameters are scaled by args.bsz)"
    if gaussians._parameters.is_cuda:
        with _lib.host_region("batch_total"):
            return _train_one_batch_hbm(gaussians, scene, batched_cameras, parameters_grad_buffer,
                                        background, pipe_args, comm_stream, args)
    return _train_one_batch_host(gaussians, scene, batched_cameras, parameters_grad_buffer,
                                 background, pipe_args, comm_stream, perm_generator, args)


def clm_offload_eval_one_cam(camera, gaussians, background, scene, render_mode="RGB", return_alpha=False):
    with torch.no_grad():
        a_ = utils.get_args()
        dp_partial = bool(getattr(gaussians, "lazy_rows", False) and dp.active()
                          and (getattr(a_, "dp_owner_computes", False) or getattr(a_, "dp_locality", False)))
        if dp_partial:
            gaussians.flush_lazy_rows()
        if getattr(gaussians, "small_deferred", False):
            gaussians.flush_small()
        filters, _, _ = calculate_filters([camera], gaussians.get_xyz, gaussians.get_opacity,
                                          gaussians.get_scaling, gaussians.get_rotation)
        f = filters[0]
        if getattr(gaussians, "lazy_rows", False):
            if not getattr(gaussians, "moments_sharded", False):
                gaussians.catch_up_rows(f.to(torch.int32))
        if getattr(gaussians, "deferred_host_rows", False):
            gaussians.host_rows_prepare(f.to(torch.int32).cpu().contiguous(), None)
        xyz = gaussians._xyz.detach()[f]
        opa = gaussians.opacity_activation(gaussians._opacity.detach()[f])
        sca = gaussians.scaling_activation(gaussians._scaling.detach()[f])
        rot = gaussians.rotation_activation(gaussians._rotation.detach()[f])
        shs = torch.empty((f.shape[0], 48), device=xyz.device)
        send_shs2gpu_stream(shs, gaussians._parameters.data, f)
        res = pipeline_forward_one_step(opa, sca, rot, xyz, shs, camera, scene, gaussians,
                                        background, None, eval=True, render_mode=render_mode,
                                        return_alpha=return_alpha)
    return res[0] if render_mode == "RGB" else (res[0],) + tuple(res[3:])
```

### include/clmgs.h

```cpp
#ifndef CLMGS_H
#define CLMGS_H
#include <stddef.h>
#include <stdint.h>

#ifdef __cplusplus
extern "C" {
#endif

#define CLMGS_EINVAL 10001
#define CLMGS_ENOMEM 10002

int clmgs_version(void);
const char* clmgs_last_error(void);

int clmgs_projection_fwd(void* stream, int C, int N, const float* means, const float* quats,
                         const float* scales, const float* viewmats, const float* Ks, int width,
                         int height, float eps2d, float near_plane, float far_plane,
                         float radius_clip, int32_t* radii, float* means2d, float* depths,
                         float* conics);
int clmgs_visibility_raw(void* stream, int C, int N, const float* means, const float* quats_raw,
                         const float* log_scales, const float* viewmats, const float* Ks, int width,
                         int height, float eps2d, float near_plane, float far_plane,
                         float radius_clip, int32_t* radii);

size_t clmgs_visibility_select_temp_bytes(int C, int N);
int clmgs_visibility_select_count(void* stream, int C, int N, const float* means,
                                  const float* quats_raw, const float* log_scales,
                                  const float* viewmats, const float* Ks, int width, int height,
                                  float eps2d, float near_plane, float far_plane, float radius_clip,
                                  void* temp, size_t temp_bytes, int64_t* cum_totals);
int clmgs_visibility_select_count_blocks(void* stream, int C, int N, const float* means, const float* quats_raw,
                                         const float* log_scales, const float* viewmats, const float* Ks, int width,
                                         int height, float eps2d, float near_plane, float far_plane, float radius_clip,
                                         void* temp, size_t temp_bytes, int64_t* cum_totals,
                                         const uint8_t* block_flags);
int clmgs_visibility_select_emit(void* stream, int C, int N, const void* temp, int64_t* out);
int clmgs_projection_bwd(void* stream, int C, int N, const float* means, const float* quats,
                         const float* scales, const float* viewmats, const float* Ks, int width,
                         int height, float eps2d, const int32_t* radii, const float* v_means2d,
                         const float* v_depths, const float* v_conics, float* v_means,
                         float* v_quats, float* v_scales);

int clmgs_sh_fwd(void* stream, int n, int degree, const float* dirs, const float* coeffs,
                 const uint8_t* masks, float* colors);
int clmgs_sh_bwd(void* stream, int n, int degree, const float* dirs, const float* coeffs,
                 const uint8_t* masks, const float* v_colors, float* v_coeffs, int accumulate,
                 float* v_dirs);

size_t clmgs_isect_count_temp_bytes(int CN);
int clmgs_isect_count(void* stream, int C, int N, const float* means2d, const int32_t* radii,
                      int tile_size, int tile_width, int tile_height, int32_t* tiles_per_gauss,
                      int64_t* cum, void* temp, size_t temp_bytes);
size_t clmgs_isect_sort_temp_bytes(int64_t n_isects);
int clmgs_isect_emit_sort(void* stream, int C, int N, int64_t n_isects, const float* means2d,
                          const int32_t* radii, const float* depths, const int64_t* cum,
                          int tile_size, int tile_width, int tile_height, int64_t* isect_ids,
                          int32_t* flatten_ids, void* temp, size_t temp_bytes);
int clmgs_isect_offsets(void* stream, int64_t n_isects, const int64_t* isect_ids, int C,
                        int tile_width, int tile_height, int32_t* offsets);

size_t clmgs_isect2_order_temp_bytes(int V);
int clmgs_isect2_order_count(void* stream, int V, const float* means2d, const int32_t* radii,
                             const float* depths, int tile_size, int tile_width, int tile_height,
                             const void* packed, int32_t* order, int64_t* cum, uint64_t* boxes,
                             int64_t* totals, void* temp, size_t temp_bytes, int64_t* row_cum);
size_t clmgs_isect2_sort_temp_bytes(int64_t n_isects);
int clmgs_isect2_emit_sort(void* stream, int V, int64_t n_isects, const float* depths,
                           const int32_t* order, const int64_t* cum, const uint64_t* boxes,
                           int tile_width, int tile_height, int32_t* flatten_ids, int32_t* offsets,
                           int64_t* isect_ids, int32_t* emit_slot, void* temp, size_t temp_bytes,
                           const int64_t* row_cum);

size_t clmgs_rasterize_pack_bytes(int C, int N);
int clmgs_rasterize_fwd(void* stream, int C, int N, int64_t n_isects, const float* means2d,
                        const float* conics, const float* colors, const float* opacities,
                        const float* backgrounds, int width, int height, int tile_size,
                        int tile_width, int tile_height, const int32_t* offsets,
                        const int32_t* flatten_ids, void* packed, float* render_colors,
                        float* render_alphas, int32_t* last_ids);
size_t clmgs_rasterize_partials_bytes(int64_t n_isects);
int clmgs_rasterize_bwd(void* stream, int C, int N, int64_t n_isects, const void* packed,
                        const float* backgrounds, int width, int height, int tile_size,
                        int tile_width, int tile_height, const int32_t* offsets,
                        const int32_t* flatten_ids, const float* render_alphas,
                        const int32_t* last_ids, const float* v_render_colors,
                        const float* v_render_alphas, void* packed_grad, float* v_means2d,
                        float* v_conics, float* v_colors, float* v_opacities,
                        const int32_t* emit_slot, const int64_t* row_cum, void* partials);

int clmgs_rasterize4_fwd(void* stream, int C, int N, int64_t n_isects, const float* means2d,
                         const float* conics, const float* colors, const float* opacities,
                         const float* backgrounds, int width, int height, int tile_size,
                         int tile_width, int tile_height, const int32_t* offsets,
                         const int32_t* flatten_ids, void* packed, float* render_colors,
                         float* render_alphas, int32_t* last_ids);
int clmgs_rasterize4_bwd(void* stream, int C, int N, int64_t n_isects, const void* packed,
                         const float* backgrounds, int width, int height, int tile_size,
                         int tile_width, int tile_height, const int32_t* offsets,
                         const int32_t* flatten_ids, const float* render_alphas,
                         const int32_t* last_ids, const float* v_render_colors,
                         const float* v_render_alphas, void* packed_grad, float* v_means2d,
                         float* v_conics, float* v_colors, float* v_opacities,
                         const int32_t* emit_slot, const int64_t* row_cum, void* partials);

int clmgs_isect2_emit_sort_dev(void* stream, int V, int64_t capacity, const int64_t* n_isects_dev,
                               const float* depths, const int32_t* order, const int64_t* cum,
                               const uint64_t* boxes, int tile_width, int tile_height,
                               int32_t* flatten_ids, int32_t* offsets, int64_t* isect_ids,
                               int32_t* emit_slot, void* temp, size_t temp_bytes, const int64_t* row_cum);

size_t clmgs_isect3_front_temp_bytes(int V, int n_tiles);
int clmgs_isect3_front(void* stream, int V, const float* means2d, const int32_t* radii, int tile_size, int tile_width,
                       int tile_height, const void* packed, int64_t* totals, int64_t* row_cum, void* temp,
                       size_t temp_bytes);
size_t clmgs_isect3_bin_temp_bytes(int64_t n_isects, int n_tiles);
int clmgs_isect3_bin(void* stream, int V, int64_t n_isects, const float* depths, int tile_width, int tile_height,
                     const int64_t* row_cum, const void* front_temp, int32_t* flatten_ids, int32_t* offsets,
                     int64_t* isect_ids, int32_t* emit_slot, void* temp, size_t temp_bytes);
int clmgs_isect3_bin_dev(void* stream, int V, int64_t capacity, const int64_t* n_isects_dev, const float* depths,
                         int tile_width, int tile_height, const int64_t* row_cum, const void* front_temp,
                         int32_t* flatten_ids, int32_t* offsets, int64_t* isect_ids, int32_t* emit_slot, void* temp,
                         size_t temp_bytes);
int clmgs_rasterize_fwd_dev(void* stream, int C, int N, int64_t capacity, const int64_t* n_isects_dev,
                            const float* backgrounds, int width, int height, int tile_size,
                            int tile_width, int tile_height, const int32_t* offsets,
                            const int32_t* flatten_ids, void* packed, float* render_colors,
                            float* render_alphas, int32_t* last_ids);
int clmgs_rasterize_bwd_dev(void* stream, int C, int N, int64_t capacity, const int64_t* n_isects_dev,
                            const void* packed, const float* backgrounds, int width, int height,
                            int tile_size, int tile_width, int tile_height, const int32_t* offsets,
                            const int32_t* flatten_ids, const float* render_alphas,
                            const int32_t* last_ids, const float* v_render_colors,
                            const float* v_render_alphas, const int32_t* emit_slot,
                            const int64_t* row_cum, void* partials);

int clmgs_preprocess_fwd(void* stream, int V, const int64_t* filter, const float* xyz,
                         const float* opacity_raw, const float* scaling_raw,
                         const float* rotation_raw, const float* sh_rows, int sh_by_filter,
                         const float* viewmat_host, const float* K_host, const float* campos_host,
                         int width, int height, int degree, float eps2d, float near_plane,
                         float far_plane, float radius_clip, int32_t* radii, float* means2d,
                         float* depths, float* conics, float* colors, float* opacities, void* packed,
                         const int32_t* sh_index);
int clmgs_preprocess_bwd(void* stream, int V, const int64_t* filter, const float* xyz,
                         const float* opacity_raw, const float* scaling_raw,
                         const float* rotation_raw, const float* sh_rows, int sh_by_filter,
                         const float* viewmat_host, const float* K_host, const float* campos_host,
                         int width, int height, int degree, float eps2d, const int32_t* radii,
                         const void* packed_grad, float* g_xyz, float* g_opacity, float* g_scaling,
                         float* g_rotation, float* g_sh_rows, float* max_radii2D, float* grad_accum,
                         float* denom, float* v_means2d_out, int stats_only_visible,
                         const void* partials, const int64_t* row_cum, const int32_t* sh_index,
                         int32_t* sh_stamp, int cur_step);

int clmgs_ssim_fwd(void* stream, int B, int CH, int H, int W, const float* img1,
                   const float* img2, float* ssim_sum, float* dm_dmu1, float* dm_dsigma1_sq,
                   float* dm_dsigma12);
int clmgs_ssim_bwd(void* stream, int B, int CH, int H, int W, const float* img1,
                   const float* img2, const float* v_mean, float inv_numel, const float* dm_dmu1,
                   const float* dm_dsigma1_sq, const float* dm_dsigma12, float* v_img1);

int clmgs_loss_slots(void);
int clmgs_l1_ssim_loss_fwd(void* stream, int H, int W, const float* img, int64_t stride_c,
                           int64_t stride_y, int64_t stride_x, const uint8_t* gt_u8,
                           float* partials, float* m1, float* m2, float* m3);
int clmgs_l1_ssim_loss_bwd(void* stream, int H, int W, const float* img, int64_t stride_c,
                           int64_t stride_y, int64_t stride_x, const uint8_t* gt_u8,
                           const float* v_loss, float lambda_dssim, const float* m1,
                           const float* m2, const float* m3, float* v_img);

int clmgs_rows_gather(void* stream, float* dst, const float* src, const void* dst_idx,
                      const void* src_idx, int idx_is_64, int64_t n_rows, int cols,
                      int grid_blocks);
int clmgs_rows_scatter_add(void* stream, float* dst, const float* src, const void* dst_idx,
                           const void* src_idx, int idx_is_64, int64_t n_rows, int cols,
                           int grid_blocks);

int clmgs_scatter_to_bit(void* stream, void* bitmap, int elem_bytes, const int64_t* filter,
                         int64_t n, int bit);
int clmgs_extract_ffs(void* stream, const void* bitmap, int elem_bytes, int64_t N, uint8_t* ffs);
int clmgs_pair_overlap_count(void* stream, const void* bitmap, int elem_bytes, int64_t N,
                             int bsz, int32_t* cnt);
int clmgs_set_signal(void* stream, int32_t* signal_pinned, int idx, int32_t value);

int clmgs_adam_rows(void* stream, float* p, float* g, float* m, float* v, const void* rows,
                    int idx_is_64, const uint8_t* mask, int64_t n_rows, int cols,
                    const float* col_lr, double beta1, double beta2, double eps, int step,
                    int bias_correction, float grad_scale, int zero_grad);
int clmgs_pack_small(void* stream, int64_t n, const float* xyz, const float* opacity,
                     const float* scaling, const float* rotation, void* packed_p);
int clmgs_adam_small_packed(void* stream, int64_t n, float* const* params, float* const* exp_avg,
                            float* const* exp_avg_sq, const double* lr4, void* packed_p,
                            void* packed_g, double beta1, double beta2, double eps, int step,
                            int bias_correction, float grad_scale, const int32_t* g_stamp, int cur_step);
int clmgs_adam_catch_up(void* stream, float* p, float* m, float* v, const int32_t* last_step,
                        const void* rows, int idx_is_64, int64_t n_rows, int cols,
                        const float* col_lr, double beta1, double beta2, double eps, int to_step,
                        int bias_correction, int max_replay, float* g, const int32_t* g_step,
                        float grad_scale, int keep_grad);
int clmgs_host_adam_rows(float* p, float* g, float* m, float* v, const int32_t* rows,
                         int64_t n_rows, int cols, const float* col_lr, double beta1,
                         double beta2, double eps, int step, int bias_correction, float grad_scale,
                         int zero_grad, const volatile int32_t* signal, int n_threads);

int clmgs_host_pool_start(int n_threads);
int clmgs_host_usable_cpus(void);
int clmgs_memcpy_async(void* stream, void* dst, const void* src, size_t bytes, int kind);
int clmgs_host_rows_prepare(float* p, const float* g, float* m, float* v, int32_t* last_step,
                            int32_t* g_step, const int32_t* rows, int64_t n_rows, int cols,
                            const float* col_lr, double beta1, double beta2, double eps, int to_step,
                            int next_g_step, int bias_correction, float grad_scale, int max_replay,
                            float* stage, int sparse);

int clmgs_densify_stats(void* stream, int64_t n, const int64_t* filter, const float* v_means2d,
                        const int32_t* radii, int only_visible, float half_w, float half_h,
                        float* max_radii2D,
                        float* xyz_gradient_accum, float* denom);

size_t clmgs_morton_order_temp_bytes(int64_t n);
int clmgs_morton_order(void* stream, int64_t n, const float* xyz, const double* lo_hi, int64_t* order, void* temp,
                       size_t temp_bytes);

int clmgs_tsp_tour(int n, const int64_t* dist, int32_t* tour);

int clmgs_knn3_mean_dist2(void* stream, int n, const float* pts_sorted, const int32_t* cell_start,
                          float ox, float oy, float oz, float h, int gx, int gy, int gz,
                          int max_ring, float* mean_d2_sorted);

size_t clmgs_host_groups_temp_bytes(int64_t n);
int clmgs_host_groups(void* stream, int64_t n, const int64_t* touched, const void* bitmap, int elem_bytes, int bsz,
                      const uint8_t* staged, int slot0, int32_t* late_sorted, int32_t* rows_by_last, int32_t* slot_of,
                      int64_t* counts, void* temp, size_t temp_bytes);

int clmgs_publish_pack(void* stream, float* msg, const float* table, const int64_t* own_rows, const int32_t* stamp,
                       int step, int64_t lo, int64_t n_rows, int64_t chunk, int cols);

int clmgs_visibility_candidates(void* stream, int C, int N, int own_lo, int own_hi, const float* means,
                                const float* log_scales, const float* viewmats, const float* Ks, int width,
                                int height, float eps2d, float near_plane, float far_plane, float pos_margin,
                                float scale_gain, uint8_t* mask);
int clmgs_small_rows_scatter(void* stream, int64_t n_rows, const int64_t* rows, const void* lines, float* xyz,
                             float* opacity, float* scaling, float* rotation, void* packed_p);
int clmgs_adam_small_packed_range(void* stream, int64_t n, int64_t row_begin, int64_t row_end, float* const* params,
                                  float* const* exp_avg, float* const* exp_avg_sq, const double* lr4, void* packed_p,
                                  void* packed_g, double beta1, double beta2, double eps, int step,
                                  int bias_correction, float grad_scale, const int32_t* g_stamp, int cur_step);

int clmgs_small_deferred_kmax(void);
int clmgs_adam_small_deferred(void* stream, int64_t n, float* const* params, float* const* exp_avg,
                              float* const* exp_avg_sq, void* packed_p, const void* packed_g, const int32_t* g_stamp,
                              int32_t* blk_last, int to_step, int n_hist, const double* lr4_hist,
                              const int32_t* step_index, const float* pos_margin, const float* scale_gain, double beta1,
                              double beta2, double eps, float grad_scale, int C, const float* viewmats, const float* Ks,
                              int width, int height, float eps2d, float near_plane, float far_plane, int flush_all,
                              uint8_t* blk_flag );

int clmgs_device_errors(uint32_t* bits, int reset);

void* clmgs_pinned_alloc(size_t bytes);
int clmgs_pinned_free(void* p);

#ifdef __cplusplus
}
#endif
#endif
```

### profiles/loss_microbench.py

```python
import sys
import torch
sys.path.insert(0, ".")
from clm_gs_amd import _lib
from clm_gs_amd._lib import check, dptr, stream
W, H = (int(sys.argv[1]), int(sys.argv[2])) if len(sys.argv) > 2 else (4608, 3456)
L = _lib.lib()
dev = "cuda"
g = torch.Generator(device=dev).manual_seed(0)
base = torch.rand((3, H, W), device=dev, generator=g)
gt = (torch.rand((3, H, W), device=dev, generator=g) * 255).to(torch.uint8)
maps = torch.empty((3, 3, H, W), device=dev)
one = torch.ones(1, device=dev)
res = {}
for name in ("planar", "interleaved"):
    if name == "planar":
        img = base.clone(); sc, sy, sx = H * W, W, 1
    else:
        img = base.permute(1, 2, 0).contiguous(); sc, sy, sx = 1, 3 * W, 3
    v_img = torch.empty_like(img)
    part = torch.zeros((L.clmgs_loss_slots(), 2), device=dev)
    def fwd():
        check(L.clmgs_l1_ssim_loss_fwd(stream(), H, W, dptr(img), sc, sy, sx, dptr(gt, torch.uint8), dptr(part),
                                       dptr(maps[0]), dptr(maps[1]), dptr(maps[2])))
    def bwd():
        check(L.clmgs_l1_ssim_loss_bwd(stream(), H, W, dptr(img), sc, sy, sx, dptr(gt, torch.uint8), dptr(one), 0.2,
                                       dptr(maps[0]), dptr(maps[1]), dptr(maps[2]), dptr(v_img)))
    for f, nm in ((fwd, "fwd"), (bwd, "bwd")):
        for _ in range(3):
            f()
        torch.cuda.synchronize()
        a, b = torch.cuda.Event(enable_timing=True), torch.cuda.Event(enable_timing=True)
        a.record()
        for _ in range(20):
            f()
        b.record()
        torch.cuda.synchronize()
        res[f"{name}_{nm}_ms"] = round(a.elapsed_time(b) / 20, 4)
    res[f"{name}_loss"] = (part.sum(0) / (23.0 * 3 * H * W)).tolist()
    res[f"{name}_vsum"] = float(v_img.double().abs().sum())
print(res)
```

### profiles/make_pmc_json.py

```python
import ast
import json
import re
import sys

GROUPS = {
    "clmgs_rasterize_bwd": ["rasterize_bwd_kernel"],
    "clmgs_rasterize_fwd": ["rasterize_fwd_kernel"],
    "clmgs_l1_ssim_loss_fwd": ["loss_fwd_kernel"],
    "clmgs_l1_ssim_loss_bwd": ["loss_bwd_kernel"],
    "clmgs_preprocess_fwd": ["preprocess_fwd_kernel"],
    "clmgs_preprocess_bwd": ["preprocess_bwd_kernel"],
    "clmgs_adam_rows": ["adam_rows_kernel"],
    "clmgs_adam_catch_up": ["adam_catch_up"],
    "clmgs_adam_small_deferred": ["adam_small_deferred_kernel"],
    "clmgs_isect3_front": ["isect3_rows_kernel", "isect3_rows_finish_kernel"],
    "clmgs_isect3_bin": ["isect3_tile_scan_kernel", "isect3_scatter_kernel", "isect3_sort_"],
}


MEDIAN_KERNELS = ("adam_catch_up",)


def _lines(path):
    rows = []
    for line in open(path):
        m = re.match(r"(.*?) (\{.*?\}) launches (\d+)(?: median (\{.*\}))?", line.strip())
        if m:
            mean = ast.literal_eval(m.group(2))
            med = ast.literal_eval(m.group(4)) if m.group(4) else mean
            rows.append((m.group(1), mean, med, int(m.group(3))))
    for x in MEDIAN_KERNELS:
        fam = [r for r in rows if x in r[0]]
        if len(fam) > 1:
            keep = max(fam, key=lambda r: r[3])
            rows = [r for r in rows if r not in fam or r is keep]
    for name, mean, med, _n in rows:
        yield name, (med if any(x in name for x in MEDIAN_KERNELS) else mean)


def read(path, counter):
    return {k: d[counter] * 1024.0 for k, d in _lines(path) if counter in d}


def read_raw(path, counter):
    return {k: d[counter] for k, d in _lines(path) if counter in d}


f, w = read(sys.argv[1], "FETCH_SIZE"), read(sys.argv[2], "WRITE_SIZE")
sq = read_raw(sys.argv[3], "SQ_INSTS_VALU") if len(sys.argv) > 3 else {}
label = sys.argv[4] if len(sys.argv) > 4 else "this round's build"
algo = {}
if len(sys.argv) > 5:
    for line in open(sys.argv[5]):
        if line.startswith("{"):
            j = json.loads(line)
            for name, k in (j.get("kernels") or {}).items():
                if "algo_GBps" in k:
                    algo[name] = k["algo_GBps"] * 1e9 * k["avg_ms"] * 1e-3
            rf = j.get("roofline") or {}
            if rf.get("kernel") and rf.get("algo_bytes_per_launch"):
                algo[rf["kernel"]] = rf["algo_bytes_per_launch"]
res = {"_note": "rocprofv3 --pmc FETCH_SIZE / WRITE_SIZE (separate passes, --kernel-trace only), KB per launch "
                "averaged over the launches of `bench.py --steps 1 --warmup 1`; bytes = KB*1024, summed over "
                "the device kernels of one C-ABI call. MI355X guide: FETCH_SIZE reports 1/2 of wide coalesced "
                "reads on gfx950 (x2 applied in fetch_bytes_x2); other widths and WRITE_SIZE uncalibrated. "
                "traffic = fetch_bytes_x2 + write_bytes.",
       "rubble28m": {}}
for entry, kernels in GROUPS.items():
    fr = sum(v for k, v in f.items() if any(x in k for x in kernels) and "unsigned long" not in k)
    wr = sum(v for k, v in w.items() if any(x in k for x in kernels) and "unsigned long" not in k)
    if fr + wr == 0:
        continue
    res["rubble28m"][entry] = {"fetch_bytes_raw": fr, "fetch_bytes_x2": 2 * fr, "write_bytes": wr,
                               "traffic": 2 * fr + wr}
    if entry in algo:
        res["rubble28m"][entry]["algo_bytes"] = round(algo[entry], 1)
        res["rubble28m"][entry]["traffic_over_algo"] = round((2 * fr + wr) / algo[entry], 3)
    if any(x in k for k in list(f) + list(w) for x in kernels if x in MEDIAN_KERNELS):
        res["rubble28m"][entry]["launch"] = "median launch of the per-camera passes (split_catch_up: four per batch; the whole-table flush excluded)"
    vi = sum(v for k, v in sq.items() if any(x in k for x in kernels) and "unsigned long" not in k)
    if vi:
        res["rubble28m"][entry]["valu_insts"] = vi
res["_source"] = "rocprofv3 --pmc passes of " + label + " (profiles/collect_r06.sh)"
json.dump(res, open(__file__.replace("make_pmc_json.py", "pmc_traffic.json"), "w"), indent=1)
print(json.dumps(res["rubble28m"], indent=1))
```

### profiles/timeline_streams.py

```python
import sqlite3
import sys

db = sys.argv[1]
arg = sys.argv[2] if len(sys.argv) > 2 else "31"
c = sqlite3.connect(db)
rows = list(c.execute("select name, start, end, queue_id, grid_x, workgroup_x, lds_size from kernels order by start"))
if arg.startswith("step"):
    marks = [r[1] for r in rows if "visibility_bits" in r[0]]
    k = int(arg[4:] or 2)
    t0, t_end = marks[-k - 1], marks[-k]
    rows = [r for r in rows if t0 <= r[1] < t_end]
else:
    t_end = max(r[2] for r in rows)
    t0 = t_end - float(arg) * 1e6
    rows = [r for r in rows if r[1] >= t0]
KEYS = ("rasterize_bwd", "rasterize_fwd", "partials_sum", "preprocess_bwd", "preprocess_fwd", "loss_bwd",
        "loss_fwd", "adam_rows", "adam_small", "catch_up", "radix_scan_rows", "radix_scatter",
        "radix_onesweep", "radix_hist_all", "radix_hist", "radix_scan_digits", "isect2_keys", "isect2_count",
        "isect2_emit", "isect2_offsets", "scan_i64_blocks", "scan_i64_totals", "scan_i64_add",
        "visibility_bits", "visibility_emit", "copyBuffer", "fillBuffer", "index_put", "direct_copy")


def short(n):
    n = n.split("(")[0]
    for k in KEYS:
        if k in n:
            return k
    return n[-28:]


queues = sorted(set(r[3] for r in rows))
print("queues:", queues)
for n, s, e, q, gx, wx, lds in rows:
    print(f"{(s - t0) / 1e6:8.3f} {(e - s) / 1e3:8.1f}us  q{queues.index(q)}  {short(n):18s} grid {gx // max(wx, 1)}x{wx} lds {lds}")
print()
raster_q = None
for q in queues:
    mine = [r for r in rows if r[3] == q]
    busy = sum(r[2] - r[1] for r in mine)
    n_r = sum(1 for r in mine if "rasterize" in r[0])
    print(f"q{queues.index(q)}: {len(mine)} kernels, busy {busy / 1e6:.2f} ms, tile kernels {n_r}")
    if n_r and (raster_q is None or n_r > raster_q[1]):
        raster_q = (q, n_r)
if raster_q:
    q = raster_q[0]
    mine = [r for r in rows if r[3] == q]
    print(f"\nidle gaps of q{queues.index(q)} (tile kernels) > 50 us and the other queues' kernels inside them:")
    for a, b in zip(mine[:-1], mine[1:]):
        gap = b[1] - a[2]
        if gap > 50e3:
            inside = [r for r in rows if r[3] != q and r[2] > a[2] and r[1] < b[1]]
            desc = ", ".join(f"{short(r[0])}:{(min(r[2], b[1]) - max(r[1], a[2])) / 1e3:.0f}" for r in inside)
            print(f"  {gap / 1e3:7.0f} us after {short(a[0])} at {(a[2] - t0) / 1e6:.2f} ms: {desc}")
```

Before: 201.4.

## Fuse L1+SSIM loss forward and backward into one strip kernel

Replaces the separate loss forward (which wrote three derivative maps) and backward kernels with a single templated kernel. It computes the SSIM partial derivatives in a register/LDS ring and convolves them on the fly to emit the image gradient directly, using overlapping strips with a wider halo. This removes the HBM round trip for the 3x3xHxW maps, one kernel launch, and the mem-stream scratch reservation. In exchange it recomputes halo columns and rows across strips, raises register/LDS pressure, and changes strip height and prefetch depth. The autograd backward now scales a precomputed gradient by the incoming cotangent.

```diff
diff --git a/clm_gs_amd/_lib.py b/clm_gs_amd/_lib.py
--- a/clm_gs_amd/_lib.py
+++ b/clm_gs_amd/_lib.py
@@ -50,8 +50,8 @@
     "clmgs_ssim_fwd": (_i, [_vp, _i, _i, _i, _i, _vp, _vp, _vp, _vp, _vp, _vp]),
     "clmgs_ssim_bwd": (_i, [_vp, _i, _i, _i, _i, _vp, _vp, _vp, _f, _vp, _vp, _vp, _vp]),
     "clmgs_loss_slots": (_i, []),
-    "clmgs_l1_ssim_loss_fwd": (_i, [_vp, _i, _i, _vp, _i64, _i64, _i64, _vp, _vp, _vp, _vp, _vp]),
-    "clmgs_l1_ssim_loss_bwd": (_i, [_vp, _i, _i, _vp, _i64, _i64, _i64, _vp, _vp, _f, _vp, _vp, _vp, _vp]),
+    "clmgs_loss_strip_rows": (_i, []),
+    "clmgs_l1_ssim_loss": (_i, [_vp, _i, _i, _vp, _i64, _i64, _i64, _vp, _f, _vp, _vp]),
     "clmgs_rows_gather": (_i, [_vp, _vp, _vp, _vp, _vp, _i, _i64, _i, _i]),
     "clmgs_rows_scatter_add": (_i, [_vp, _vp, _vp, _vp, _vp, _i, _i64, _i, _i]),
     "clmgs_scatter_to_bit": (_i, [_vp, _vp, _i, _vp, _i64, _i]),
@@ -118,7 +118,7 @@
     pass
 
 
-_NO_STREAM = {"clmgs_version", "clmgs_loss_slots", "clmgs_small_deferred_kmax", "clmgs_isect3_front_temp_bytes",
+_NO_STREAM = {"clmgs_version", "clmgs_loss_slots", "clmgs_loss_strip_rows", "clmgs_small_deferred_kmax", "clmgs_isect3_front_temp_bytes",
               "clmgs_isect3_bin_temp_bytes", "clmgs_last_error", "clmgs_isect_count_temp_bytes",
               "clmgs_isect_sort_temp_bytes", "clmgs_host_groups_temp_bytes", "clmgs_isect2_order_temp_bytes", "clmgs_isect2_sort_temp_bytes", "clmgs_visibility_select_temp_bytes", "clmgs_rasterize_pack_bytes", "clmgs_rasterize_partials_bytes", "clmgs_host_adam_rows", "clmgs_host_pool_start", "clmgs_host_usable_cpus", "clmgs_host_rows_prepare", "clmgs_tsp_tour",
               "clmgs_pinned_alloc", "clmgs_pinned_free", "clmgs_device_errors"}
diff --git a/clm_gs_amd/clm_kernels.py b/clm_gs_amd/clm_kernels.py
--- a/clm_gs_amd/clm_kernels.py
+++ b/clm_gs_amd/clm_kernels.py
@@ -53,32 +53,21 @@
         need = image.requires_grad
         slots = L.clmgs_loss_slots()
         partials = torch.zeros((slots, 2), dtype=F32, device=image.device)
-        maps = torch.empty((3, 3, H, W), dtype=F32, device=image.device) if need else None
+        v_img = torch.empty_strided(image.shape, image.stride(), dtype=F32, device=image.device) if need else None
         sc, sy, sx = image.stride()
-        check(L.clmgs_l1_ssim_loss_fwd(stream(), H, W, ctypes.c_void_p(image.data_ptr()), sc, sy, sx,
-                                       dptr(gt_u8, U8), dptr(partials),
-                                       dptr(maps[0] if need else None, F32, True),
-                                       dptr(maps[1] if need else None, F32, True),
-                                       dptr(maps[2] if need else None, F32, True)))
+        check(L.clmgs_l1_ssim_loss(stream(), H, W, ctypes.c_void_p(image.data_ptr()), sc, sy, sx,
+                                   dptr(gt_u8, U8), float(lambda_dssim), dptr(partials),
+                                   ctypes.c_void_p(v_img.data_ptr()) if need else None))
         tot = partials.sum(dim=0) / float(image.numel())
-        ctx.lam = float(lambda_dssim)
+        lam = float(lambda_dssim)
         if need:
-            ctx.save_for_backward(image, gt_u8, maps)
-        return (1.0 - ctx.lam) * tot[0] + ctx.lam * (1.0 - tot[1])
+            ctx.save_for_backward(v_img)
+        return (1.0 - lam) * tot[0] + lam * (1.0 - tot[1])
 
     @staticmethod
     def backward(ctx, v):
-        L = _lib.lib()
-        image, gt_u8, maps = ctx.saved_tensors
-        _, H, W = image.shape
-        v = v.reshape(1).to(F32).contiguous()
-        v_img = torch.empty_strided(image.shape, image.stride(), dtype=F32, device=image.device)
-        sc, sy, sx = image.stride()
-        check(L.clmgs_l1_ssim_loss_bwd(stream(), H, W, ctypes.c_void_p(image.data_ptr()), sc, sy, sx,
-                                       dptr(gt_u8, U8), dptr(v, F32), ctx.lam, dptr(maps[0]),
-                                       dptr(maps[1]), dptr(maps[2]),
-                                       ctypes.c_void_p(v_img.data_ptr())))
-        return v_img, None, None
+        v_img, = ctx.saved_tensors
+        return v.to(F32) * v_img, None, None
 
 
 def fused_l1_ssim_loss(image, gt_u8, lambda_dssim=0.2):
diff --git a/clm_gs_amd/csrc/loss.hip b/clm_gs_amd/csrc/loss.hip
--- a/clm_gs_amd/csrc/loss.hip
+++ b/clm_gs_amd/csrc/loss.hip
@@ -4,17 +4,26 @@
 
 constexpr int LR = 5;
 constexpr int LM = 2 * LR + 1;
-constexpr int LS_W = 64, LS_ROWS = 62;
+#ifndef CLMGS_LOSS_ROWS
+#define CLMGS_LOSS_ROWS 124
+#endif
+constexpr int LS_W = 64, LS_ROWS = CLMGS_LOSS_ROWS;
 constexpr int LS_IN = LS_W + 2 * LR;
 constexpr int LS_PITCH = LS_IN + 2;
-constexpr int LS_RING = 8;
 constexpr int LU = 12;
 #ifndef CLMGS_LOSS_LP
-#define CLMGS_LOSS_LP 4
+#define CLMGS_LOSS_LP 2
 #endif
 constexpr int LP = CLMGS_LOSS_LP;
 constexpr int LOSS_SLOTS = 1024;
 constexpr float L_C1 = 0.01f * 0.01f, L_C2 = 0.03f * 0.03f;
+static_assert(LU % LP == 0 && LU > 2 * LR, "the register rings hold a whole window");
+
+template <bool GRAD> struct LossStrip {
+  static constexpr int OW = GRAD ? LS_W - 2 * LR : LS_W;
+  static constexpr int PAD = GRAD ? 2 * LR : LR;
+  static constexpr int RING = GRAD ? 16 : 8;
+};
 
 constexpr float l_win[11] = {
     0.0010283801f, 0.0075987582f, 0.0360007721f, 0.1093606895f, 0.2130055377f, 0.2660117249f,
@@ -35,109 +44,181 @@
   return fmaf(fmaf(-q, 255.0f, v), r, q);
 }
 
+template <int OW>
 __device__ __forceinline__ bool strip_of_block(int H, int W, int& c, int& x0, int& y0, int& slot) {
-  const int n_sx = (W + LS_W - 1) / LS_W, n_sy = (H + LS_ROWS - 1) / LS_ROWS;
+  const int n_sx = (W + OW - 1) / OW, n_sy = (H + LS_ROWS - 1) / LS_ROWS;
   const int grp = blockIdx.x / 24, rem = blockIdx.x - grp * 24;
   c = rem >> 3;
   const int strip = grp * 8 + (rem & 7);
   if (strip >= n_sx * n_sy) return false;
   const int by = strip / n_sx, bx = strip - by * n_sx;
-  x0 = bx * LS_W; y0 = by * LS_ROWS;
+  x0 = bx * OW; y0 = by * LS_ROWS;
   slot = ((c * n_sy + by) * n_sx + bx) & (LOSS_SLOTS - 1);
   return true;
 }
 
-#ifndef CLMGS_LOSS_FWD_WAVES
-#define CLMGS_LOSS_FWD_WAVES 3
+
+struct LossIn {
+  const float* img_c; const uint8_t* gt_c; int64_t sy;
+  int H, W, y_first, n_rows;
+  unsigned xs_c, xh_c, xs_off, xh_off;
+};
+struct LossRow { float a, ha; unsigned b, hb; };
+
+__device__ __forceinline__ void loss_fetch(const LossIn& in, int r, LossRow& p) {
+  const int y = min(max(in.y_first + min(r, in.n_rows - 1), 0), in.H - 1);
+  const float* ir = in.img_c + y * in.sy;
+  const uint8_t* gr = in.gt_c + (size_t)y * in.W;
+  p.a = ir[in.xs_off]; p.b = gr[in.xs_c];
+  p.ha = ir[in.xh_off]; p.hb = gr[in.xh_c];
+}
+
+__device__ __forceinline__ void loss_row_to_lds(float* la, float* lb, int lane, const LossRow& p, bool okm, bool okh) {
+  la[lane] = okm ? p.a : 0.f; lb[lane] = okm ? gt_from_byte(p.b) : 0.f;
+  if (lane < 2 * LR) {
+    la[LS_W + lane] = okh ? p.ha : 0.f; lb[LS_W + lane] = okh ? gt_from_byte(p.hb) : 0.f;
+  }
+}
+
+__device__ __forceinline__ void loss_hsum4(const float* la, const float* lb, int lane, float (&o)[4]) {
+  float s0 = 0.f, s1 = 0.f, s2 = 0.f, s3 = 0.f;
+#pragma unroll
+  for (int j = 0; j < LM; ++j) {
+    const float av = la[lane + j], bv = lb[lane + j];
+    const float wa_ = l_win[j] * av, wb_ = l_win[j] * bv;
+    s0 += wa_; s1 += wb_; s2 = fmaf(wa_, av, s2); s2 = fmaf(wb_, bv, s2); s3 = fmaf(wa_, bv, s3);
+  }
+  o[0] = s0; o[1] = s1; o[2] = s2; o[3] = s3;
+}
+
+__device__ __forceinline__ void loss_hsum3(const float (&lm)[3][LS_PITCH], int lane, float (&o)[3]) {
+  float s0 = 0.f, s1 = 0.f, s2 = 0.f;
+#pragma unroll
+  for (int j = 0; j < LM; ++j) {
+    s0 = fmaf(l_win[j], lm[0][lane + j], s0);
+    s1 = fmaf(l_win[j], lm[1][lane + j], s1);
+    s2 = fmaf(l_win[j], lm[2][lane + j], s2);
+  }
+  o[0] = s0; o[1] = s1; o[2] = s2;
+}
+
+template <int N>
+__device__ __forceinline__ void loss_vsum(const float (&win)[LU][N], int k, float (&o)[N]) {
+#pragma unroll
+  for (int q = 0; q < N; ++q) {
+    float sacc = 0.f;
+#pragma unroll
+    for (int j = 0; j < LM; ++j) sacc = fmaf(l_win[j], win[(k + 2 + j) % LU][q], sacc);
+    o[q] = sacc;
+  }
+}
+
+struct SsimPoint { float val, mu1, mu2, A, B, D, E, iDE; };
+__device__ __forceinline__ SsimPoint loss_ssim_point(const float (&acc)[4]) {
+  SsimPoint s;
+  s.mu1 = acc[0]; s.mu2 = acc[1];
+  const float mu1sq = s.mu1 * s.mu1, mu2sq = s.mu2 * s.mu2, mu12 = s.mu1 * s.mu2;
+  const float sgs = (acc[2] - mu1sq) - mu2sq, sg12 = acc[3] - mu12;
+  s.A = 2.f * mu12 + L_C1; s.B = 2.f * sg12 + L_C2;
+  s.D = mu1sq + mu2sq + L_C1; s.E = sgs + L_C2;
+  s.iDE = __builtin_amdgcn_rcpf(s.D * s.E);
+  s.val = s.A * s.B * s.iDE;
+  return s;
+}
+
+__device__ __forceinline__ void loss_ssim_derivs(const SsimPoint& s, float (&d)[3]) {
+  const float d_mu1 = 2.f * s.mu2 * s.B * s.iDE - s.val * 2.f * s.mu1 * __builtin_amdgcn_rcpf(s.D);
+  const float d_s1 = -s.val * __builtin_amdgcn_rcpf(s.E), d_s12 = 2.f * s.A * s.iDE;
+  d[0] = d_mu1 - 2.f * s.mu1 * d_s1 - s.mu2 * d_s12; d[1] = d_s1; d[2] = d_s12;
+}
+
+__device__ __forceinline__ float loss_cotangent(float xv, float yv, const float (&g)[3], float w_l1_over_numel,
+                                                float w_ssim_over_numel) {
+  const float sgn = (xv > yv) ? 1.f : ((xv < yv) ? -1.f : 0.f);
+  const float dss = g[0] + 2.f * xv * g[1] + yv * g[2];
+  return w_l1_over_numel * sgn - w_ssim_over_numel * dss;
+}
+
+#ifndef CLMGS_LOSS_WAVES
+#define CLMGS_LOSS_WAVES 3
 #endif
-__global__ void __launch_bounds__(64, CLMGS_LOSS_FWD_WAVES)
-loss_fwd_kernel(int H, int W, ImgView img, const uint8_t* __restrict__ gt, float* __restrict__ partials,
-                float* __restrict__ m1, float* __restrict__ m2, float* __restrict__ m3) {
-  __shared__ float la[LS_RING][LS_PITCH], lb[LS_RING][LS_PITCH];
+template <bool GRAD>
+__global__ void __launch_bounds__(64, GRAD ? CLMGS_LOSS_WAVES : 3)
+loss_kernel(int H, int W, ImgView img, const uint8_t* __restrict__ gt, float* __restrict__ partials,
+            float w_l1_over_numel, float w_ssim_over_numel, float* __restrict__ v_img) {
+  using S = LossStrip<GRAD>;
+  constexpr int PAD = S::PAD, RING = S::RING;
+  __shared__ float la[RING][LS_PITCH], lb[RING][LS_PITCH];
+  __shared__ float lm[GRAD ? 2 : 1][3][LS_PITCH];
   const int lane = threadIdx.x;
   int c, x0, y0, slot;
-  if (!strip_of_block(H, W, c, x0, y0, slot)) return;
+  if (!strip_of_block<S::OW>(H, W, c, x0, y0, slot)) return;
   const size_t plane = (size_t)H * W;
+  const int n_out = min(LS_ROWS, H - y0);
+  const int n_rows = n_out + 2 * PAD;
+  const int xs = x0 - PAD + lane;
+  const bool xs_ok = xs >= 0 && xs < W;
+  const int xh = xs + LS_W;
+  const bool h_ok = lane < 2 * LR && xh < W;
+  const int xm = xs + LR;
+  const bool xm_ok = xm >= 0 && xm < W;
+  const bool xm_own = xm_ok && xm >= x0 && xm < x0 + S::OW;
   const int xo = x0 + lane;
-  const int n_rows = min(LS_ROWS, H - y0) + 2 * LR;
-  const int xs = x0 - LR + lane;
-  const bool xs_ok = xs >= 0 && xs < W;
-  const int xh = x0 - LR + LS_W + lane;
-  const bool h_ok = lane < 2 * LR && xh < W;
-  const float* img_c = img.p + c * img.sc;
-  const uint8_t* gt_c = gt + c * plane;
-  const unsigned xs_c = (unsigned)min(max(xs, 0), W - 1);
-  const unsigned xh_c = (unsigned)min(x0 - LR + LS_W + min(lane, 2 * LR - 1), W - 1);
-  const unsigned xs_off = xs_c * (unsigned)img.sx, xh_off = xh_c * (unsigned)img.sx;
-  float pa[LP], ha[LP];
-  unsigned pb[LP], hb[LP];
-  auto fetch = [&](int r, int s) {
-    const int y = min(max(y0 - LR + min(r, n_rows - 1), 0), H - 1);
-    const float* ir = img_c + y * img.sy;
-    const uint8_t* gr = gt_c + (size_t)y * W;
-    pa[s] = ir[xs_off]; pb[s] = gr[xs_c];
-    ha[s] = ir[xh_off]; hb[s] = gr[xh_c];
-  };
-#pragma unroll
-  for (int s = 0; s < LP; ++s) fetch(s, s);
-  float win[LU][4];
+  const bool xo_ok = lane < S::OW && xo < W;
+  LossIn in;
+  in.img_c = img.p + c * img.sc; in.gt_c = gt + c * plane; in.sy = img.sy;
+  in.H = H; in.W = W; in.y_first = y0 - PAD; in.n_rows = n_rows;
+  in.xs_c = (unsigned)min(max(xs, 0), W - 1);
+  in.xh_c = (unsigned)min(x0 - PAD + LS_W + min(lane, 2 * LR - 1), W - 1);
+  in.xs_off = in.xs_c * (unsigned)img.sx; in.xh_off = in.xh_c * (unsigned)img.sx;
+  const unsigned xo_voff = (unsigned)xo * (unsigned)img.sx;
+  LossRow pf[LP];
+#pragma unroll
+  for (int s = 0; s < LP; ++s) loss_fetch(in, s, pf[s]);
+  float win[LU][4] = {};
+  float wing[LU][GRAD ? 3 : 1] = {};
   float l1 = 0.f, ss = 0.f;
   for (int r0 = 0; r0 < n_rows; r0 += LU) {
 #pragma unroll
     for (int k = 0; k < LU; ++k) {
       const int r = r0 + k;
+      __builtin_amdgcn_sched_barrier(0);
+      const int s = k % LP, buf = r & (RING - 1);
       {
-        __builtin_amdgcn_sched_barrier(0);
-        const int s = k % LP, buf = r & (LS_RING - 1);
-        {
-          const int yin = y0 - LR + r;
-          const bool row_ok = yin >= 0 && yin < H;
-          const bool okm = row_ok && xs_ok, okh = row_ok && h_ok;
-          la[buf][lane] = okm ? pa[s] : 0.f; lb[buf][lane] = okm ? gt_from_byte(pb[s]) : 0.f;
-          if (lane < 2 * LR) {
-            la[buf][LS_W + lane] = okh ? ha[s] : 0.f; lb[buf][LS_W + lane] = okh ? gt_from_byte(hb[s]) : 0.f;
-          }
-        }
-        fetch(r + LP, s);
+        const int yin = y0 - PAD + r;
+        const bool row_ok = yin >= 0 && yin < H;
+        loss_row_to_lds(la[buf], lb[buf], lane, pf[s], row_ok && xs_ok, row_ok && h_ok);
+      }
+      loss_fetch(in, r + LP, pf[s]);
+      wave_sync();
+      loss_hsum4(la[buf], lb[buf], lane, win[k]);
+      float acc[4];
+      loss_vsum<4>(win, k, acc);
+      const SsimPoint sp = loss_ssim_point(acc);
+      const int ym = y0 - PAD + r - LR;
+      const bool ym_ok = r >= 2 * LR && ym >= 0 && ym < H;
+      const bool sum_ok = ym_ok && ym >= y0 && ym < y0 + n_out && xm_own;
+      ss += sum_ok ? sp.val : 0.f;
+      const int cbuf = (r - LR) & (RING - 1);
+      l1 += sum_ok ? fabsf(la[cbuf][lane + LR] - lb[cbuf][lane + LR]) : 0.f;
+      if constexpr (!GRAD) {
+        asm volatile("" : "+v"(ss), "+v"(l1));
+      } else {
+        float d[3];
+        loss_ssim_derivs(sp, d);
+        const bool okm = ym_ok && xm_ok;
+        float (&lmr)[3][LS_PITCH] = lm[r & 1];
+        lmr[0][lane] = okm ? d[0] : 0.f; lmr[1][lane] = okm ? d[1] : 0.f; lmr[2][lane] = okm ? d[2] : 0.f;
         wave_sync();
-        float s0 = 0.f, s1 = 0.f, s2 = 0.f, s3 = 0.f;
-#pragma unroll
-        for (int j = 0; j < LM; ++j) {
-          const float av = la[buf][lane + j], bv = lb[buf][lane + j];
-          const float wa_ = l_win[j] * av, wb_ = l_win[j] * bv;
-          s0 += wa_; s1 += wb_; s2 = fmaf(wa_, av, s2); s2 = fmaf(wb_, bv, s2); s3 = fmaf(wa_, bv, s3);
-        }
-        win[k][0] = s0; win[k][1] = s1; win[k][2] = s2; win[k][3] = s3;
-        {
-          float acc[4];
-#pragma unroll
-          for (int q = 0; q < 4; ++q) {
-            float sacc = 0.f;
-#pragma unroll
-            for (int j = 0; j < LM; ++j) sacc += l_win[j] * win[(k + 2 + j) % LU][q];
-            acc[q] = sacc;
-          }
-          const int y = y0 + r - 2 * LR;
-          const bool out_ok = (r >= 2 * LR) && (r < n_rows) && (xo < W) && (y < H);
-          {
-            const float mu1 = acc[0], mu2 = acc[1];
-            const float mu1sq = mu1 * mu1, mu2sq = mu2 * mu2, mu12 = mu1 * mu2;
-            const float sgs = (acc[2] - mu1sq) - mu2sq, sg12 = acc[3] - mu12;
-            const float A = 2.f * mu12 + L_C1, B = 2.f * sg12 + L_C2;
-            const float D = mu1sq + mu2sq + L_C1, E = sgs + L_C2;
-            const float iDE = __builtin_amdgcn_rcpf(D * E);
-            const float val = A * B * iDE;
-            ss += out_ok ? val : 0.f;
-            const int cbuf = (r - LR) & (LS_RING - 1);
-            l1 += out_ok ? fabsf(la[cbuf][lane + LR] - lb[cbuf][lane + LR]) : 0.f;
-            if (m1 && out_ok) {
-              const float d_mu1 = 2.f * mu2 * B * iDE - val * 2.f * mu1 * __builtin_amdgcn_rcpf(D);
-              const float d_s1 = -val * __builtin_amdgcn_rcpf(E), d_s12 = 2.f * A * iDE;
-              const size_t orow = c * plane + (size_t)y * W;
-              (m1 + orow)[(unsigned)xo] = d_mu1 - 2.f * mu1 * d_s1 - mu2 * d_s12;
-              (m2 + orow)[(unsigned)xo] = d_s1; (m3 + orow)[(unsigned)xo] = d_s12;
-            }
-          }
+        loss_hsum3(lmr, lane, wing[k]);
+        float g[3];
+        loss_vsum<3>(wing, k, g);
+        const int obuf = (r - 2 * LR) & (RING - 1);
+        const float xv = la[obuf][lane + 2 * LR], yv = lb[obuf][lane + 2 * LR];
+        if (r >= 2 * PAD && r < n_rows && xo_ok) {
+          const int yo = y0 + r - 2 * PAD;
+          (v_img + (c * img.sc + yo * img.sy))[xo_voff] =
+              loss_cotangent(xv, yv, g, w_l1_over_numel, w_ssim_over_numel);
         }
       }
     }
@@ -149,133 +230,30 @@
   }
 }
 
-#ifndef CLMGS_LOSS_BWD_WAVES
-#define CLMGS_LOSS_BWD_WAVES 3
-#endif
-__global__ void __launch_bounds__(64, CLMGS_LOSS_BWD_WAVES)
-loss_bwd_kernel(int H, int W, ImgView img, const uint8_t* __restrict__ gt, const float* __restrict__ v,
-                float w_l1_over_numel, float w_ssim_over_numel, const float* __restrict__ m1,
-                const float* __restrict__ m2, const float* __restrict__ m3, float* __restrict__ v_img,
-                int64_t vsc, int64_t vsy, int64_t vsx) {
-  __shared__ float lm[2][3][LS_PITCH];
-  const int lane = threadIdx.x;
-  int c, x0, y0, slot;
-  if (!strip_of_block(H, W, c, x0, y0, slot)) return;
-  const size_t plane = (size_t)H * W;
-  const int xo = x0 + lane;
-  const int n_out = min(LS_ROWS, H - y0);
-  const int n_rows = n_out + 2 * LR;
-  const int xs = x0 - LR + lane;
-  const bool xs_ok = xs >= 0 && xs < W;
-  const int hg = lane >> 4, hl = lane & 15;
-  const int xh = x0 - LR + LS_W + hl;
-  const bool h_ok = hg < 3 && hl < 2 * LR && xh < W;
-  const float* mh = (hg == 0 ? m1 : (hg == 1 ? m2 : m3)) + c * plane;
-  const float* m1c = m1 + c * plane;
-  const float* m2c = m2 + c * plane;
-  const float* m3c = m3 + c * plane;
-  const float* img_c = img.p + c * img.sc;
-  const uint8_t* gt_c = gt + c * plane;
-  const float vv = v[0];
-  const unsigned xs_c = (unsigned)min(max(xs, 0), W - 1);
-  const unsigned xh_c = (unsigned)min(x0 - LR + LS_W + min(hl, 2 * LR - 1), W - 1);
-  const unsigned xo_c = (unsigned)min(xo, W - 1);
-  const unsigned xo_off = xo_c * (unsigned)img.sx;
-  const unsigned xo_voff = (unsigned)xo * (unsigned)vsx;
-  float p1[LP], p2[LP], p3[LP], ph[LP], px[LP];
-  unsigned py[LP];
-  auto fetch = [&](int r, int s) {
-    const int rc = min(r, n_rows - 1);
-    const int y = min(max(y0 - LR + rc, 0), H - 1);
-    const int yo = min(max(y0 + rc - 2 * LR, 0), H - 1);
-    const size_t o = (size_t)y * W;
-    p1[s] = (m1c + o)[xs_c]; p2[s] = (m2c + o)[xs_c]; p3[s] = (m3c + o)[xs_c];
-    ph[s] = (mh + o)[xh_c];
-    px[s] = (img_c + yo * img.sy)[xo_off];
-    py[s] = (gt_c + (size_t)yo * W)[xo_c];
-  };
-#pragma unroll
-  for (int s = 0; s < LP; ++s) fetch(s, s);
-  float win[LU][3];
-  for (int r0 = 0; r0 < n_rows; r0 += LU) {
-#pragma unroll
-    for (int k = 0; k < LU; ++k) {
-      const int r = r0 + k;
-      {
-        __builtin_amdgcn_sched_barrier(0);
-        const int s = k % LP, buf = r & 1;
-        {
-          const int yin = y0 - LR + r;
-          const bool row_ok = yin >= 0 && yin < H;
-          const bool okm = row_ok && xs_ok;
-          lm[buf][0][lane] = okm ? p1[s] : 0.f; lm[buf][1][lane] = okm ? p2[s] : 0.f; lm[buf][2][lane] = okm ? p3[s] : 0.f;
-          if (hg < 3 && hl < 2 * LR) lm[buf][hg][LS_W + hl] = (row_ok && h_ok) ? ph[s] : 0.f;
-        }
-        const float xv = px[s], yv = gt_from_byte(py[s]);
-        fetch(r + LP, s);
-        wave_sync();
-        float s0 = 0.f, s1 = 0.f, s2 = 0.f;
-#pragma unroll
-        for (int j = 0; j < LM; ++j) {
-          s0 = fmaf(l_win[j], lm[buf][0][lane + j], s0);
-          s1 = fmaf(l_win[j], lm[buf][1][lane + j], s1);
-          s2 = fmaf(l_win[j], lm[buf][2][lane + j], s2);
-        }
-        win[k][0] = s0; win[k][1] = s1; win[k][2] = s2;
-        {
-          float g[3];
-#pragma unroll
-          for (int q = 0; q < 3; ++q) {
-            float sacc = 0.f;
-#pragma unroll
-            for (int j = 0; j < LM; ++j) sacc += l_win[j] * win[(k + 2 + j) % LU][q];
-            g[q] = sacc;
-          }
-          const int y = y0 + r - 2 * LR;
-          if (r >= 2 * LR && r < n_rows && xo < W) {
-            const float sgn = (xv > yv) ? 1.f : ((xv < yv) ? -1.f : 0.f);
-            const float dss = g[0] + 2.f * xv * g[1] + yv * g[2];
-            (v_img + (c * vsc + y * vsy))[xo_voff] = vv * (w_l1_over_numel * sgn - w_ssim_over_numel * dss);
-          }
-        }
-        wave_sync();
-      }
-    }
-  }
-}
-
 }
 
 using namespace clmgs;
 
 extern "C" int clmgs_loss_slots(void) { return LOSS_SLOTS; }
-
-extern "C" int clmgs_l1_ssim_loss_fwd(void* stream, int H, int W, const float* img, int64_t stride_c,
-                                      int64_t stride_y, int64_t stride_x, const uint8_t* gt_u8,
-                                      float* partials, float* m1, float* m2, float* m3) {
+extern "C" int clmgs_loss_strip_rows(void) { return LS_ROWS; }
+
+template <bool GRAD>
+static void loss_launch(hipStream_t stream, int H, int W, ImgView v, const uint8_t* gt_u8, float lambda_dssim,
+                        float* partials, float* v_img) {
+  const double numel = 3.0 * (double)H * (double)W;
+  const int64_t strips = (int64_t)ceil_div(W, LossStrip<GRAD>::OW) * ceil_div(H, LS_ROWS);
+  dim3 grid((unsigned)(24 * ceil_div(strips, 8)));
+  hipLaunchKernelGGL(loss_kernel<GRAD>, grid, dim3(64), 0, stream, H, W, v, gt_u8, partials,
+                     (float)((1.0 - lambda_dssim) / numel), (float)(lambda_dssim / numel), v_img);
+}
+
+extern "C" int clmgs_l1_ssim_loss(void* stream, int H, int W, const float* img, int64_t stride_c,
+                                  int64_t stride_y, int64_t stride_x, const uint8_t* gt_u8,
+                                  float lambda_dssim, float* partials, float* v_img) {
   CLMGS_CHECK_ARG(H >= 1 && W >= 1 && img && gt_u8 && partials);
-  CLMGS_CHECK_ARG((m1 && m2 && m3) || (!m1 && !m2 && !m3));
   ImgView v{img, stride_c, stride_y, stride_x};
-  const int64_t strips = (int64_t)ceil_div(W, LS_W) * ceil_div(H, LS_ROWS);
-  dim3 grid((unsigned)(24 * ceil_div(strips, 8)));
-  hipLaunchKernelGGL(loss_fwd_kernel, grid, dim3(64), 0, (hipStream_t)stream, H, W, v, gt_u8,
-                     partials, m1, m2, m3);
+  if (v_img) loss_launch<true>((hipStream_t)stream, H, W, v, gt_u8, lambda_dssim, partials, v_img);
+  else loss_launch<false>((hipStream_t)stream, H, W, v, gt_u8, lambda_dssim, partials, nullptr);
   CLMGS_LAUNCH_CHECK();
   return 0;
 }
-
-extern "C" int clmgs_l1_ssim_loss_bwd(void* stream, int H, int W, const float* img, int64_t stride_c,
-                                      int64_t stride_y, int64_t stride_x, const uint8_t* gt_u8,
-                                      const float* v_loss, float lambda_dssim, const float* m1,
-                                      const float* m2, const float* m3, float* v_img) {
-  CLMGS_CHECK_ARG(H >= 1 && W >= 1 && img && gt_u8 && v_loss && m1 && m2 && m3 && v_img);
-  ImgView v{img, stride_c, stride_y, stride_x};
-  const double numel = 3.0 * (double)H * (double)W;
-  const int64_t strips = (int64_t)ceil_div(W, LS_W) * ceil_div(H, LS_ROWS);
-  dim3 grid((unsigned)(24 * ceil_div(strips, 8)));
-  hipLaunchKernelGGL(loss_bwd_kernel, grid, dim3(64), 0, (hipStream_t)stream, H, W, v, gt_u8, v_loss,
-                     (float)((1.0 - lambda_dssim) / numel), (float)(lambda_dssim / numel), m1, m2, m3,
-                     v_img, stride_c, stride_y, stride_x);
-  CLMGS_LAUNCH_CHECK();
-  return 0;
-}
diff --git a/clm_gs_amd/fused.py b/clm_gs_amd/fused.py
--- a/clm_gs_amd/fused.py
+++ b/clm_gs_amd/fused.py
@@ -47,7 +47,7 @@
 class _CameraPass:
     __slots__ = ("V", "cam", "filt", "sh_rows", "sh_by_filter", "small_in", "small_packed", "radii",
                  "packed", "fids", "offsets", "emit_slot", "row_cum", "out", "alphas", "last_ids",
-                 "bg", "v_out", "maps", "loss", "ev_loss", "streams", "deg", "aux", "loss_partials",
+                 "bg", "v_out", "loss", "ev_loss", "streams", "deg", "aux", "loss_partials",
                  "lambda_dssim", "gt_u8", "background", "isect", "sh_index", "means2d", "n_dev")
 
 
@@ -181,27 +181,17 @@
     with torch.cuda.stream(s_mem):
         slots = L.clmgs_loss_slots()
         partials = torch.zeros((slots, 2), dtype=F32, device=dev)
-        maps = p.maps = torch.empty((3, 3, H, W), dtype=F32, device=dev)
         sc, sy, sx = 1, 3 * W, 3
         gt = gt_u8.contiguous()
-        sm = _sptr(s_mem)
-        check(L.clmgs_l1_ssim_loss_fwd(sm, H, W, dptr(p.out), sc, sy, sx, dptr(gt, U8), dptr(partials),
-                                       dptr(maps[0]), dptr(maps[1]), dptr(maps[2])))
+        p.v_out = torch.empty_like(p.out)
+        check(L.clmgs_l1_ssim_loss(_sptr(s_mem), H, W, dptr(p.out), sc, sy, sx, dptr(gt, U8), float(lambda_dssim),
+                                   dptr(partials), dptr(p.v_out)))
         p.loss_partials, p.loss = partials, None
-        one = getattr(gaussians, "_clmgs_one", None)
-        if one is None or one.device != dev:
-            one = gaussians._clmgs_one = torch.ones((1,), dtype=F32, device=dev)
-        p.v_out = torch.empty_like(p.out)
-        check(L.clmgs_l1_ssim_loss_bwd(sm, H, W, dptr(p.out), sc, sy, sx, dptr(gt, U8), dptr(one),
-                                       float(lambda_dssim), dptr(maps[0]), dptr(maps[1]), dptr(maps[2]),
-                                       dptr(p.v_out)))
         p.ev_loss = None
         if s_raster is not s_mem:
             p.ev_loss = torch.cuda.Event()
             p.ev_loss.record(s_mem)
-        p.aux = p.aux + (gt, one, partials)
-        p.maps = None
-        del maps
+        p.aux = p.aux + (gt, partials)
     return p
 
 
diff --git a/clm_gs_amd/strategies/clm_offload/engine.py b/clm_gs_amd/strategies/clm_offload/engine.py
--- a/clm_gs_amd/strategies/clm_offload/engine.py
+++ b/clm_gs_amd/strategies/clm_offload/engine.py
@@ -203,7 +203,7 @@
     sts = _pipeline_streams(gaussians)
     plan = {
         "front": (sts["mem"][0], k * (20 * P + 70 * I + 96 * V)),
-        "mem": (sts["mem"][1], k * 48 * P + (1 << 20)),
+        "mem": (sts["mem"][1], k * 12 * P + (1 << 20)),
         "raster": (sts["raster"][0], 2 * k * 64 * int(0.8 * I)),
         "default": (torch.cuda.current_stream(), 240 * N + 64 * V * 4),
     }
@@ -414,8 +414,6 @@
     gaussians, bsz, step = b.gaussians, b.bsz, b.step
     sts = _pipeline_streams(gaussians)
     s_front, s_mem, s_raster = sts["mem"][0], sts["mem"][1], sts["raster"][0]
-    if getattr(gaussians, "_clmgs_one", None) is None:
-        gaussians._clmgs_one = torch.ones((1,), dtype=torch.float32, device=b.params.device)
     for st_ in (s_front, s_mem, s_raster):
         st_.wait_stream(b.default_stream)
     gaussians._clmgs_passes = None
diff --git a/include/clmgs.h b/include/clmgs.h
--- a/include/clmgs.h
+++ b/include/clmgs.h
@@ -161,13 +161,10 @@
                    const float* dm_dsigma1_sq, const float* dm_dsigma12, float* v_img1);
 
 int clmgs_loss_slots(void);
-int clmgs_l1_ssim_loss_fwd(void* stream, int H, int W, const float* img, int64_t stride_c,
-                           int64_t stride_y, int64_t stride_x, const uint8_t* gt_u8,
-                           float* partials, float* m1, float* m2, float* m3);
-int clmgs_l1_ssim_loss_bwd(void* stream, int H, int W, const float* img, int64_t stride_c,
-                           int64_t stride_y, int64_t stride_x, const uint8_t* gt_u8,
-                           const float* v_loss, float lambda_dssim, const float* m1,
-                           const float* m2, const float* m3, float* v_img);
+int clmgs_loss_strip_rows(void);
+int clmgs_l1_ssim_loss(void* stream, int H, int W, const float* img, int64_t stride_c,
+                       int64_t stride_y, int64_t stride_x, const uint8_t* gt_u8,
+                       float lambda_dssim, float* partials, float* v_img);
 
 int clmgs_rows_gather(void* stream, float* dst, const float* src, const void* dst_idx,
                       const void* src_idx, int idx_is_64, int64_t n_rows, int cols,
diff --git a/profiles/loss_microbench.py b/profiles/loss_microbench.py
--- a/profiles/loss_microbench.py
+++ b/profiles/loss_microbench.py
@@ -9,9 +9,7 @@
 g = torch.Generator(device=dev).manual_seed(0)
 base = torch.rand((3, H, W), device=dev, generator=g)
 gt = (torch.rand((3, H, W), device=dev, generator=g) * 255).to(torch.uint8)
-maps = torch.empty((3, 3, H, W), device=dev)
-one = torch.ones(1, device=dev)
-res = {}
+res = {"strip_rows": L.clmgs_loss_strip_rows()}
 for name in ("planar", "interleaved"):
     if name == "planar":
         img = base.clone(); sc, sy, sx = H * W, W, 1
@@ -19,23 +17,28 @@
         img = base.permute(1, 2, 0).contiguous(); sc, sy, sx = 1, 3 * W, 3
     v_img = torch.empty_like(img)
     part = torch.zeros((L.clmgs_loss_slots(), 2), device=dev)
-    def fwd():
-        check(L.clmgs_l1_ssim_loss_fwd(stream(), H, W, dptr(img), sc, sy, sx, dptr(gt, torch.uint8), dptr(part),
-                                       dptr(maps[0]), dptr(maps[1]), dptr(maps[2])))
-    def bwd():
-        check(L.clmgs_l1_ssim_loss_bwd(stream(), H, W, dptr(img), sc, sy, sx, dptr(gt, torch.uint8), dptr(one), 0.2,
-                                       dptr(maps[0]), dptr(maps[1]), dptr(maps[2]), dptr(v_img)))
-    for f, nm in ((fwd, "fwd"), (bwd, "bwd")):
+    def grad():
+        check(L.clmgs_l1_ssim_loss(stream(), H, W, dptr(img), sc, sy, sx, dptr(gt, torch.uint8), 0.2, dptr(part),
+                                   dptr(v_img)))
+    def value():
+        check(L.clmgs_l1_ssim_loss(stream(), H, W, dptr(img), sc, sy, sx, dptr(gt, torch.uint8), 0.2, dptr(part),
+                                   None))
+    n_calls = 0
+    for f, nm, reps in ((grad, "grad", 5), (value, "value", 1)):
         for _ in range(3):
             f()
         torch.cuda.synchronize()
-        a, b = torch.cuda.Event(enable_timing=True), torch.cuda.Event(enable_timing=True)
-        a.record()
-        for _ in range(20):
-            f()
-        b.record()
-        torch.cuda.synchronize()
-        res[f"{name}_{nm}_ms"] = round(a.elapsed_time(b) / 20, 4)
-    res[f"{name}_loss"] = (part.sum(0) / (23.0 * 3 * H * W)).tolist()
+        ms = []
+        for _ in range(reps):
+            a, b = torch.cuda.Event(enable_timing=True), torch.cuda.Event(enable_timing=True)
+            a.record()
+            for _ in range(20):
+                f()
+            b.record()
+            torch.cuda.synchronize()
+            ms.append(round(a.elapsed_time(b) / 20, 4))
+        n_calls += 3 + 20 * reps
+        res[f"{name}_{nm}_ms"] = ms
+    res[f"{name}_loss"] = (part.sum(0) / (n_calls * 3.0 * H * W)).tolist()
     res[f"{name}_vsum"] = float(v_img.double().abs().sum())
 print(res)
diff --git a/profiles/make_pmc_json.py b/profiles/make_pmc_json.py
--- a/profiles/make_pmc_json.py
+++ b/profiles/make_pmc_json.py
@@ -6,8 +6,7 @@
 GROUPS = {
     "clmgs_rasterize_bwd": ["rasterize_bwd_kernel"],
     "clmgs_rasterize_fwd": ["rasterize_fwd_kernel"],
-    "clmgs_l1_ssim_loss_fwd": ["loss_fwd_kernel"],
-    "clmgs_l1_ssim_loss_bwd": ["loss_bwd_kernel"],
+    "clmgs_l1_ssim_loss": ["loss_kernel"],
     "clmgs_preprocess_fwd": ["preprocess_fwd_kernel"],
     "clmgs_preprocess_bwd": ["preprocess_bwd_kernel"],
     "clmgs_adam_rows": ["adam_rows_kernel"],
diff --git a/profiles/timeline_streams.py b/profiles/timeline_streams.py
--- a/profiles/timeline_streams.py
+++ b/profiles/timeline_streams.py
@@ -14,8 +14,8 @@
     t_end = max(r[2] for r in rows)
     t0 = t_end - float(arg) * 1e6
     rows = [r for r in rows if r[1] >= t0]
-KEYS = ("rasterize_bwd", "rasterize_fwd", "partials_sum", "preprocess_bwd", "preprocess_fwd", "loss_bwd",
-        "loss_fwd", "adam_rows", "adam_small", "catch_up", "radix_scan_rows", "radix_scatter",
+KEYS = ("rasterize_bwd", "rasterize_fwd", "partials_sum", "preprocess_bwd", "preprocess_fwd", "loss_kernel",
+        "loss_bwd", "loss_fwd", "adam_rows", "adam_small", "catch_up", "radix_scan_rows", "radix_scatter",
         "radix_onesweep", "radix_hist_all", "radix_hist", "radix_scan_digits", "isect2_keys", "isect2_count",
         "isect2_emit", "isect2_offsets", "scan_i64_blocks", "scan_i64_totals", "scan_i64_add",
         "visibility_bits", "visibility_emit", "copyBuffer", "fillBuffer", "index_put", "direct_copy")
```

New measurement: 201.6 (median of 3 runs). About the same (+0.1%).
